# veronicaguerrini/BFQzip

Measured on AMD Instinct MI355X. Metric: Mbases/s end-to-end (eBWT+cluster+LF), reads and results resident in HBM, higher is better.
Workload: dtype u64

## Files before the change

bfqzip_amd/_lib.py:

```python
import ctypes as C
import os
import subprocess

_HERE = os.path.dirname(os.path.abspath(__file__))
LIB_PATH = os.path.join(_HERE, "libbfqhip.so")
_LIB = None

SYMBOLS = [
    "bfq_default_params", "bfq_create", "bfq_create_error", "bfq_destroy", "bfq_set_params",
    "bfq_last_error", "bfq_stream", "bfq_device_count", "bfq_pick_device", "bfq_device_lease", "bfq_device_release",
    "bfq_phase_enable", "bfq_phase", "bfq_phase_report", "bfq_output_prefault", "bfq_fastq_rows_estimate", "bfq_build_ebwt", "bfq_count_reads",
    "bfq_smooth_invert", "bfq_run_reads", "bfq_run_reads_device", "bfq_fetch_ebwt",
    "bfq_fastq_out_bound", "bfq_fastq_build_ebwt", "bfq_fastq_run", "bfq_fastq_run_streams",
    "bfq_smooth_invert_fastq", "bfq_fastq_run_job", "bfq_host_alloc", "bfq_host_free",
    "bfq_text_count_lines", "bfq_text_nth_newline", "bfq_file_put", "bfq_file_map", "bfq_file_unmap", "bfq_fastq_build_ebwt_fd", "bfq_smooth_invert_fastq_fd",
    "bfq_glob_begin", "bfq_glob_local_text", "bfq_glob_pile_counts", "bfq_glob_init_out", "bfq_glob_run_pile", "bfq_glob_finish",
    "bfq_synth_default", "bfq_synth_total", "bfq_synth_host", "bfq_synth_device", "bfq_synth_fastq",
    "bfq_posbin_geometry", "bfq_prof_enable", "bfq_prof_reset", "bfq_prof_count", "bfq_prof_get", "bfq_prof_trace_select", "bfq_prof_trace",
    "bfq_stream_bound", "bfq_stream_raw_len", "bfq_stream_compress", "bfq_stream_decompress",
    "bfq_stream_reserve", "bfq_stream_compress_device", "bfq_stream_ebwt_decode",
    "bfq_names_compress", "bfq_names_compress_device",
    "bfq_quals_compress", "bfq_quals_compress_device",
    "bfq_fastq_restore_bound", "bfq_fastq_restore", "bfq_fastq_restore_fd",
    "bfq_reorder_key", "bfq_fastq_reorder", "bfq_fastq_reorder_fd",
    "bfq_perm_bound", "bfq_perm_reads", "bfq_perm_encode", "bfq_perm_decode",
    "bfq_fastq_reorder_keep", "bfq_fastq_reorder_keep_fd", "bfq_fastq_unreorder", "bfq_fastq_unreorder_fd",
    "bfq_fastq_restore_ordered", "bfq_fastq_restore_ordered_fd",
    "bfq_fastq_restore_groups", "bfq_stream_members", "bfq_fastq_restore_grouped", "bfq_fastq_restore_grouped_fd",
    "bfq_fastq_compare", "bfq_fastq_compare_fd",
    "bfq_bgzf_probe", "bfq_bgzf_index", "bfq_bgzf_inflate", "bfq_bgzf_inflate_device", "bfq_bgzf_inflate_fd",
    "bfq_bgzf_deflate_bound", "bfq_bgzf_deflate_host", "bfq_bgzf_deflate", "bfq_bgzf_deflate_device", "bfq_bgzf_deflate_fd",
    "bfq_fastq_restore_bgzf_fd",
    "bfq_gzip_probe", "bfq_gzip_measure", "bfq_gzip_inflate", "bfq_gzip_inflate_device", "bfq_gzip_inflate_fd", "bfq_gzip_inflate_host",
    "bfq_gzip_host_error",
    "bfq_workspace_bytes", "bfq_version",
]


class Params(C.Structure):
    _fields_ = [(k, C.c_int32) for k in ("K", "m", "v", "f", "t", "term", "M", "B", "ext", "piles", "ws_cap_mib")] + \
               [("reserved", C.c_int32 * 5)]


class Stats(C.Structure):
    _fields_ = [(k, C.c_uint64) for k in (
        "num_clust", "num_clust_discarded", "num_clust_amb_discarded", "num_clust_mod",
        "num_clust_alleq", "bases_inside", "qs_smoothed", "modified",
        "n_rows", "n_reads", "n_segments", "n_big_segments")]

    def as_dict(self):
        return {k: int(getattr(self, k)) for k, _ in self._fields_}


class Synth(C.Structure):
    _fields_ = [("seed", C.c_uint64), ("N", C.c_uint64), ("Lmin", C.c_uint32), ("Lmax", C.c_uint32),
                ("coverage", C.c_uint32), ("err_ppm", C.c_uint32), ("n_ppm", C.c_uint32),
                ("snp_every", C.c_uint32), ("dsnp_every", C.c_uint32), ("both_strands", C.c_uint32),
                ("first", C.c_uint64), ("collection", C.c_uint64), ("reserved", C.c_uint32 * 2)]


MAX_PARTS = 4


class TextPart(C.Structure):
    _fields_ = [("data", C.c_void_p), ("len", C.c_uint64)]


class ReorderOpts(C.Structure):
    _fields_ = [("mode", C.c_int32), ("k", C.c_int32), ("seed", C.c_uint64), ("reserved", C.c_uint64 * 2)]


class RestoreGroup(C.Structure):
    _fields_ = [(k, C.c_uint64) for k in ("dna_off", "dna_len", "qs_off", "qs_len", "hdr_off", "hdr_len", "raw_stream", "raw_hdr",
                                          "reads", "text_bound")]


class BgzfMember(C.Structure):
    _fields_ = [("in_off", C.c_uint64), ("out_off", C.c_uint64), ("in_len", C.c_uint32), ("out_len", C.c_uint32)]


class GzipStats(C.Structure):
    _fields_ = [(k, C.c_uint64) for k in ("members", "pieces", "decoders", "chain", "skipped", "discarded")]

    def as_dict(self):
        return {k: int(getattr(self, k)) for k, _ in self._fields_}

    def __repr__(self):
        return "GzipStats(%s)" % ", ".join("%s=%d" % kv for kv in self.as_dict().items())


CMP_SYMS = 6
CMP_POS = 512


class CompareDiff(C.Structure):
    _fields_ = [("read", C.c_uint64), ("pos", C.c_uint32), ("base_a", C.c_uint8), ("base_b", C.c_uint8), ("qual_a", C.c_uint8), ("qual_b", C.c_uint8)]


COMPARE_SCALARS = ("n_reads", "total_bases", "n_diffs", "reads_changed", "reads_bases_changed", "reads_quals_changed", "bases_changed",
                   "quals_changed", "quals_raised", "quals_lowered", "qual_abs_sum", "qual_sq_sum", "qual_abs_max", "first_changed_read",
                   "headers_same", "headers_dropped", "headers_changed")
COMPARE_ARRAYS = (("subst", CMP_SYMS * CMP_SYMS), ("qual_hist_a", 256), ("qual_hist_b", 256), ("changed_base_qual_hist", 256),
                  ("pos_len", CMP_POS), ("pos_bases", CMP_POS), ("pos_quals", CMP_POS), ("pos_abs", CMP_POS))


class CompareReport(C.Structure):
    _fields_ = [(k, C.c_uint64) for k in COMPARE_SCALARS] + [(k, C.c_uint64 * n) for k, n in COMPARE_ARRAYS] + [("reserved", C.c_uint64 * 8)]


class FastqJob(C.Structure):
    _fields_ = [("parts", C.POINTER(TextPart)), ("nparts", C.c_int32), ("keep_headers", C.c_int32),
                ("out_fastq", C.c_void_p), ("cap_fastq", C.c_uint64),
                ("out_dna", C.c_void_p), ("out_qs", C.c_void_p), ("cap_stream", C.c_uint64),
                ("out_hdr", C.c_void_p), ("cap_hdr", C.c_uint64),
                ("fastq_len", C.c_uint64), ("stream_len", C.c_uint64), ("hdr_len", C.c_uint64),
                ("n_reads", C.c_uint64), ("total_bases", C.c_uint64),
                ("part_reads", C.c_uint64 * (MAX_PARTS + 1)), ("part_fastq_off", C.c_uint64 * (MAX_PARTS + 1)),
                ("part_stream_off", C.c_uint64 * (MAX_PARTS + 1)), ("part_hdr_off", C.c_uint64 * (MAX_PARTS + 1)),
                ("compress_streams", C.c_int32), ("name_codec", C.c_int32),
                ("dna_bytes", C.c_uint64), ("qs_bytes", C.c_uint64), ("hdr_bytes", C.c_uint64),
                ("qual_codec", C.c_int32), ("reserved1", C.c_int32)]


def build(clean=False):
    d = os.path.join(_HERE, "csrc")
    if clean:
        subprocess.check_call(["make", "-s", "-C", d, "clean"])
    subprocess.check_call(["make", "-s", "-j8", "-C", d, "all"])


def lib():
    global _LIB
    if _LIB is None:
        try:
            import torch
        except ImportError:
            pass
        if not os.path.exists(LIB_PATH):
            build()
        L = C.CDLL(LIB_PATH)
        L.bfq_create.restype = C.c_void_p
        L.bfq_create.argtypes = [C.c_int, C.POINTER(Params)]
        L.bfq_create_error.restype = C.c_char_p
        L.bfq_destroy.argtypes = [C.c_void_p]
        L.bfq_set_params.argtypes = [C.c_void_p, C.POINTER(Params)]
        L.bfq_last_error.restype = C.c_char_p
        L.bfq_last_error.argtypes = [C.c_void_p]
        L.bfq_stream.restype = C.c_void_p
        L.bfq_stream.argtypes = [C.c_void_p]
        L.bfq_version.restype = C.c_char_p
        L.bfq_workspace_bytes.restype = C.c_uint64
        L.bfq_workspace_bytes.argtypes = [C.c_void_p]
        L.bfq_synth_total.restype = C.c_uint64
        vp, u64 = C.c_void_p, C.c_uint64
        L.bfq_pick_device.argtypes = [C.c_char_p, C.c_int]
        L.bfq_device_lease.argtypes = [C.c_int, C.POINTER(C.c_char_p), C.c_int, C.c_char_p, C.c_int, C.POINTER(C.c_double)]
        L.bfq_device_release.argtypes = [C.c_int]
        L.bfq_phase_enable.argtypes = [C.c_int]
        L.bfq_phase.argtypes = [C.c_char_p]
        L.bfq_phase_report.argtypes = [C.c_char_p]
        L.bfq_output_prefault.argtypes = [C.c_int, u64, u64]
        L.bfq_fastq_rows_estimate.restype = u64
        L.bfq_fastq_rows_estimate.argtypes = [C.c_int, u64]
        L.bfq_build_ebwt.argtypes = [vp, vp, vp, vp, u64, C.c_int, vp, vp, vp]
        L.bfq_count_reads.argtypes = [vp, u64, C.c_int, C.POINTER(u64)]
        L.bfq_smooth_invert.argtypes = [vp, vp, vp, vp, C.c_int, u64, vp, vp, vp, C.POINTER(Stats)]
        L.bfq_run_reads.argtypes = [vp, vp, vp, vp, u64, vp, vp, C.POINTER(Stats)]
        L.bfq_run_reads_device.argtypes = [vp, vp, vp, vp, u64, u64, vp, vp, C.POINTER(Stats)]
        L.bfq_fetch_ebwt.argtypes = [vp, vp, vp, vp]
        L.bfq_fastq_out_bound.restype = C.c_uint64
        L.bfq_fastq_out_bound.argtypes = [u64, u64, u64]
        L.bfq_fastq_build_ebwt.argtypes = [vp, vp, u64, C.c_int, vp, vp, vp, u64, C.POINTER(u64), C.POINTER(u64)]
        L.bfq_fastq_run.argtypes = [vp, vp, u64, C.c_int, vp, u64, C.POINTER(u64), C.POINTER(Stats)]
        L.bfq_fastq_run_streams.argtypes = [vp, vp, u64, vp, vp, u64, C.POINTER(u64), vp, u64, C.POINTER(u64),
                                            C.POINTER(Stats)]
        L.bfq_smooth_invert_fastq.argtypes = [vp, vp, vp, vp, C.c_int, u64, vp, u64, vp, u64, C.POINTER(u64),
                                              C.POINTER(Stats)]
        L.bfq_fastq_run_job.argtypes = [vp, C.POINTER(FastqJob), C.POINTER(Stats)]
        L.bfq_glob_begin.argtypes = [vp, C.POINTER(TextPart), C.c_int, C.POINTER(u64), C.POINTER(u64)]
        L.bfq_glob_local_text.argtypes = [vp, vp, vp]
        L.bfq_glob_pile_counts.argtypes = [vp, vp, u64, vp]
        L.bfq_glob_init_out.argtypes = [vp, vp, vp, u64, vp, vp]
        L.bfq_glob_run_pile.argtypes = [vp, vp, vp, u64, C.c_int, C.c_int, vp, vp, C.POINTER(Stats)]
        L.bfq_glob_finish.argtypes = [vp, vp, vp, C.POINTER(FastqJob)]
        L.bfq_host_alloc.restype = vp
        L.bfq_host_alloc.argtypes = [u64]
        L.bfq_host_free.argtypes = [vp]
        L.bfq_text_count_lines.argtypes = [vp, u64, u64, vp, C.c_int]
        L.bfq_file_put.argtypes = [C.c_int, u64, vp, u64, C.c_int]
        L.bfq_file_map.restype = vp
        L.bfq_file_map.argtypes = [C.c_int, u64, u64, C.c_int]
        L.bfq_file_unmap.argtypes = [vp, u64, u64]
        L.bfq_text_nth_newline.restype = C.c_int64
        L.bfq_text_nth_newline.argtypes = [vp, u64, u64]
        L.bfq_synth_default.argtypes = [C.POINTER(Synth), u64, C.c_uint32]
        L.bfq_synth_total.argtypes = [C.POINTER(Synth)]
        L.bfq_synth_host.argtypes = [C.POINTER(Synth), vp, vp, vp]
        L.bfq_synth_device.argtypes = [vp, C.POINTER(Synth), vp, vp, vp]
        L.bfq_synth_fastq.argtypes = [vp, C.POINTER(Synth), vp, u64, C.POINTER(u64)]
        L.bfq_stream_bound.restype = u64
        L.bfq_stream_bound.argtypes = [u64]
        L.bfq_stream_raw_len.restype = C.c_int64
        L.bfq_stream_raw_len.argtypes = [vp, u64]
        L.bfq_stream_compress.argtypes = [vp, vp, u64, vp, u64, C.POINTER(u64)]
        L.bfq_stream_decompress.argtypes = [vp, vp, u64, vp, u64, C.POINTER(u64)]
        L.bfq_stream_reserve.argtypes = [vp, u64]
        L.bfq_names_compress.argtypes = [vp, vp, u64, C.c_uint32, vp, u64, C.POINTER(u64)]
        L.bfq_names_compress_device.argtypes = [vp, vp, u64, C.c_uint32, vp, u64, C.POINTER(u64)]
        L.bfq_quals_compress.argtypes = [vp, vp, u64, C.c_uint32, vp, u64, C.POINTER(u64)]
        L.bfq_quals_compress_device.argtypes = [vp, vp, u64, C.c_uint32, vp, u64, C.POINTER(u64)]
        L.bfq_stream_ebwt_decode.argtypes = [vp, vp, u64, vp, u64, vp, vp, u64, C.POINTER(u64), C.POINTER(u64)]
        L.bfq_fastq_restore_bound.restype = C.c_int64
        L.bfq_fastq_restore_bound.argtypes = [vp, u64, vp, u64, vp, u64]
        L.bfq_fastq_restore.argtypes = [vp, vp, u64, vp, u64, vp, u64, vp, u64, C.POINTER(u64), C.POINTER(u64)]
        L.bfq_fastq_restore_fd.argtypes = [vp, C.c_int, u64, C.c_int, u64, C.c_int, u64, C.c_int, C.POINTER(u64), C.POINTER(u64)]
        L.bfq_reorder_key.restype = u64
        L.bfq_reorder_key.argtypes = [vp, u64, C.c_int]
        L.bfq_fastq_reorder.argtypes = [vp, C.POINTER(TextPart), C.c_int, C.POINTER(ReorderOpts), C.POINTER(vp), C.POINTER(u64),
                                        C.POINTER(u64), vp, C.POINTER(u64)]
        L.bfq_fastq_reorder_fd.argtypes = [vp, C.POINTER(C.c_int), C.POINTER(u64), C.c_int, C.POINTER(ReorderOpts), C.POINTER(C.c_int),
                                           C.POINTER(u64), C.POINTER(u64)]
        pu64, pint = C.POINTER(u64), C.POINTER(C.c_int)
        L.bfq_perm_bound.restype = u64
        L.bfq_perm_bound.argtypes = [u64]
        L.bfq_perm_reads.restype = C.c_int64
        L.bfq_perm_reads.argtypes = [vp, u64]
        L.bfq_perm_encode.argtypes = [vp, u64, C.POINTER(ReorderOpts), vp, u64, pu64]
        L.bfq_perm_decode.argtypes = [vp, u64, vp, u64, pu64, C.POINTER(ReorderOpts), pu64]
        L.bfq_fastq_reorder_keep.argtypes = [vp, C.POINTER(TextPart), C.c_int, C.POINTER(ReorderOpts), C.POINTER(vp), pu64, pu64, vp, u64, pu64, pu64]
        L.bfq_fastq_reorder_keep_fd.argtypes = [vp, pint, pu64, C.c_int, C.POINTER(ReorderOpts), pint, C.c_int, pu64, pu64, pu64]
        L.bfq_fastq_unreorder.argtypes = [vp, C.POINTER(TextPart), C.c_int, vp, u64, C.POINTER(vp), pu64, pu64, pu64]
        L.bfq_fastq_unreorder_fd.argtypes = [vp, pint, pu64, C.c_int, C.c_int, u64, pint, pu64, pu64]
        L.bfq_fastq_restore_ordered.argtypes = [vp, vp, u64, vp, u64, vp, u64, vp, u64, vp, u64, pu64, pu64]
        L.bfq_fastq_restore_ordered_fd.argtypes = [vp, C.c_int, u64, C.c_int, u64, C.c_int, u64, C.c_int, u64, C.c_int, pu64, pu64]
        L.bfq_fastq_restore_groups.restype = C.c_int64
        L.bfq_fastq_restore_groups.argtypes = [vp, u64, vp, u64, vp, u64, C.POINTER(RestoreGroup), u64, C.c_char_p, C.c_int]
        L.bfq_stream_members.restype = C.c_int64
        L.bfq_stream_members.argtypes = [vp, u64]
        L.bfq_fastq_restore_grouped.argtypes = [vp, vp, u64, vp, u64, vp, u64, u64, u64, vp, u64, pu64, pu64]
        L.bfq_fastq_restore_grouped_fd.argtypes = [vp, C.c_int, u64, C.c_int, u64, C.c_int, u64, u64, u64, C.c_int, pu64, pu64]
        L.bfq_stream_compress_device.argtypes = [vp, vp, u64, vp, u64, C.POINTER(u64)]
        L.bfq_fastq_compare.argtypes = [vp, C.POINTER(TextPart), C.c_int, C.POINTER(TextPart), C.c_int, vp, u64, C.POINTER(CompareReport), vp, u64]
        L.bfq_fastq_compare_fd.argtypes = [vp, C.c_int, u64, C.c_int, u64, C.c_int, u64, C.POINTER(CompareReport), vp, u64]
        L.bfq_bgzf_probe.argtypes = [vp, u64]
        L.bfq_bgzf_index.argtypes = [vp, u64, C.POINTER(BgzfMember), u64, pu64, pu64, pu64]
        L.bfq_bgzf_inflate.argtypes = [vp, vp, u64, vp, u64, pu64]
        L.bfq_bgzf_inflate_device.argtypes = [vp, vp, u64, vp, u64, pu64]
        L.bfq_bgzf_inflate_fd.argtypes = [vp, C.c_int, u64, C.c_int, pu64]
        L.bfq_bgzf_deflate_bound.restype = u64
        L.bfq_bgzf_deflate_bound.argtypes = [u64]
        L.bfq_bgzf_deflate_host.argtypes = [vp, u64, C.c_int, vp, u64, pu64]
        L.bfq_bgzf_deflate.argtypes = [vp, vp, u64, C.c_int, vp, u64, pu64]
        L.bfq_bgzf_deflate_device.argtypes = [vp, vp, u64, C.c_int, vp, u64, pu64]
        L.bfq_bgzf_deflate_fd.argtypes = [vp, C.c_int, u64, C.c_int, C.c_int, pu64]
        pgs = C.POINTER(GzipStats)
        L.bfq_gzip_probe.argtypes = [vp, u64]
        L.bfq_gzip_measure.argtypes = [vp, vp, u64, u64, pu64, pu64, pgs]
        L.bfq_gzip_inflate.argtypes = [vp, vp, u64, u64, vp, u64, pu64, pgs]
        L.bfq_gzip_inflate_device.argtypes = [vp, vp, u64, u64, vp, u64, pu64, pgs]
        L.bfq_gzip_inflate_fd.argtypes = [vp, C.c_int, u64, u64, C.c_int, pu64, pgs]
        L.bfq_gzip_inflate_host.argtypes = [vp, u64, u64, vp, u64, pu64, pgs]
        L.bfq_gzip_host_error.restype = C.c_char_p
        L.bfq_gzip_host_error.argtypes = []
        L.bfq_fastq_restore_bgzf_fd.argtypes = [vp, C.c_int, u64, C.c_int, u64, C.c_int, u64, C.c_int, u64, C.c_int, C.c_int, pu64, pu64, pu64]
        L.bfq_posbin_geometry.argtypes = [u64, C.POINTER(u64), C.POINTER(C.c_int)]
        L.bfq_prof_enable.argtypes = [vp, C.c_int]
        L.bfq_prof_reset.argtypes = [vp]
        L.bfq_prof_count.argtypes = [vp]
        L.bfq_prof_trace_select.argtypes = [vp, C.c_int]
        L.bfq_prof_trace.restype = C.c_int64
        L.bfq_prof_trace.argtypes = [vp, vp, u64]
        L.bfq_prof_get.argtypes = [vp, C.c_int, C.c_char_p, C.c_int, C.POINTER(C.c_double),
                                   C.POINTER(u64), C.POINTER(C.c_double)]
        _LIB = L
    return _LIB
```

bfqzip_amd/csrc/bfq_api.hip:

```cpp
#include <math.h>
#include <time.h>
#include <stdlib.h>
#include <stdio.h>
#include <string.h>
#include <unistd.h>
#include <errno.h>
#include <algorithm>
#include <new>
#include "bfq_internal.h"
#include "bfq_synth.h"
#include "bfq_device.h"
#include "bfq_rank.h"
#include "bfq_posbin.h"

const char *const BFQ_KERNEL_NAMES[K_NUM] = {
    "k_text_from_reads", "k_pack3", "k_build_keys", "k_radix_hist", "k_scan", "k_radix_scatter", "k_huge_round",
    "k_cluster_big", "k_refine_chunk", "k_refine_big", "k_emit_bwt", "k_lf_count", "k_lf_build", "k_lcp_flags",
    "k_cluster", "k_invert_count", "k_invert", "k_synth", "k_fastq", "k_bfs", "k_codec", "misc",
    "k_restore_index", "k_fq_format_lines", "k_reorder_keys", "k_reorder_gather",
    "k_fq_format_ordered", "k_perm_pack", "k_perm_invert", "k_posbin_l1", "k_posbin_l2", "k_posbin_apply",
    "k_cmp_check", "k_cmp_compare", "k_cmp_emit", "k_bgzf_inflate", "k_bgzf_deflate"};

static thread_local std::string g_createErr;

void bfq_ctx::reserveBegin(size_t bytes)
{
    bytes = (bytes + 0xFFFFF) & ~(size_t)0xFFFFF;
    if (wsThread || bytes <= ws.cap || (wsLimit() && bytes > wsLimit())) return;
    wsPendBytes = bytes; wsPend = nullptr;
    const int dev = device;
    wsThread = new std::thread([this, dev, bytes] {
        struct timespec t0, t1;
        clock_gettime(CLOCK_MONOTONIC, &t0);
        void *p = nullptr;
        if (hipSetDevice(dev) != hipSuccess || hipMalloc(&p, bytes) != hipSuccess) { (void)hipGetLastError(); p = nullptr; }
        clock_gettime(CLOCK_MONOTONIC, &t1);
        wsPend = (char *)p;
        wsPendSecs = (t1.tv_sec - t0.tv_sec) + 1e-9 * (t1.tv_nsec - t0.tv_nsec);
    });
}
void bfq_ctx::reserveJoin(bool adopt, size_t need)
{
    if (!wsThread) return;
    wsThread->join();
    delete wsThread;
    wsThread = nullptr;
    if (!wsPend) return;
    if (adopt && need <= wsPendBytes && need > ws.cap && !(wsLimit() && wsPendBytes > wsLimit())) {
        adoptWorkspace(wsPend, wsPendBytes);
        if (bfq_env().trace) fprintf(stderr, "[bfq] workspace %.1f GiB: hipMalloc %.3f s, beside the upload\n", ws.cap / 1073741824.0, wsPendSecs);
    } else (void)hipFree(wsPend);
    wsPend = nullptr; wsPendBytes = 0;
}
void bfq_ctx::wsFree() { adoptWorkspace(nullptr, 0); }
void bfq_ctx::adoptWorkspace(char *p, size_t bytes)
{
    if (ws.base) { quiesce(); (void)hipFree(ws.base); }
    ws = Arena{p, bytes, 0, ws.peak};
}

void bfq_ctx::reserve(size_t bytes)
{
    bytes = (bytes + 0xFFFFF) & ~(size_t)0xFFFFF;
    reserveJoin(true, bytes);
    if (wsLimit() && bytes > wsLimit()) {
        char b[200];
        snprintf(b, sizeof b, "device workspace of %.1f GiB is above the cap of %.1f GiB (bfq_params.ws_cap_mib / BFQ_WS_CAP)", bytes / 1073741824.0, wsLimit() / 1073741824.0);
        throw BfqError{BFQ_E_NOMEM, b};
    }
    if (bytes > ws.cap || (wsLimit() && ws.cap > wsLimit())) {
        wsFree();
        struct timespec t0, t1;
        clock_gettime(CLOCK_MONOTONIC, &t0);
        char *p = nullptr;
        const hipError_t e = hipMalloc((void **)&p, bytes);
        clock_gettime(CLOCK_MONOTONIC, &t1);
        if (bfq_env().trace) fprintf(stderr, "[bfq] workspace %.1f GiB: hipMalloc %.3f s\n", bytes / 1073741824.0, (t1.tv_sec - t0.tv_sec) + 1e-9 * (t1.tv_nsec - t0.tv_nsec));
        if (e != hipSuccess) {
            char b[160];
            snprintf(b, sizeof b, "device workspace of %zu bytes: %s", bytes, hipGetErrorString(e));
            (void)hipGetLastError();
            throw BfqError{BFQ_E_NOMEM, b};
        }
        adoptWorkspace(p, bytes);
    }
    ws.release(0);
    d_bwt = d_qual = nullptr; d_lcp = nullptr; d_gcnt = nullptr; n = N = 0;
}
void bfq_ctx::dropWorkspace()
{
    wsFree();
    d_bwt = d_qual = nullptr; d_lcp = nullptr; d_gcnt = nullptr;
}
void bfq_ctx::profBegin(int id, double bytes)
{
    if (!profOn) return;
    if (evUsed + 2 > evPool.size()) {
        size_t old = evPool.size();
        evPool.resize(old + 256);
        for (size_t i = old; i < evPool.size(); i++) HIP_CHECK(hipEventCreate(&evPool[i]));
    }
    ProfRec r{id, evPool[evUsed], evPool[evUsed + 1], bytes};
    evUsed += 2;
    HIP_CHECK(hipEventRecord(r.a, stream));
    recs.push_back(r);
}
void bfq_ctx::profEnd()
{
    if (!profOn) return;
    HIP_CHECK(hipEventRecord(recs.back().b, stream));
}
void bfq_ctx::profCollect()
{
    for (auto &r : recs) {
        float ms = 0;
        if (hipEventElapsedTime(&ms, r.a, r.b) == hipSuccess) {
            profMs[r.id] += ms; profLaunches[r.id]++; profBytes[r.id] += r.bytes;
            if (r.id == profTraceId && profTrace.size() < (1u << 20)) profTrace.push_back(ms);
        }
    }
    recs.clear();
    evUsed = 0;
}
void bfq_ctx::sync() { HIP_CHECK(hipStreamSynchronize(stream)); }
void bfq_ctx::zeroCounters() { HIP_CHECK(hipMemsetAsync(d_cnt, 0, sizeof(DevCounters), stream)); }
void bfq_ctx::fetchCounters()
{
    HIP_CHECK(hipMemcpyAsync(&h_cnt, d_cnt, sizeof(DevCounters), hipMemcpyDeviceToHost, stream));
    sync();
}

static int host_q(double x) { return (int)round(-10 * log10(x)); }

extern "C" void bfq_default_params(bfq_params *p)
{
    memset(p, 0, sizeof(*p));
    p->K = 16; p->m = 2; p->v = '>'; p->f = 40; p->t = 20; p->term = '#'; p->M = 2; p->B = 0; p->ext = 0; p->piles = 0;
}
extern "C" const char *bfq_create_error(void) { return g_createErr.c_str(); }
extern "C" const char *bfq_version(void) { return "bfqzip_amd 0.1 (gfx950)"; }
extern "C" int bfq_device_count(void)
{
    int nd = 0;
    if (hipGetDeviceCount(&nd) != hipSuccess) { (void)hipGetLastError(); return 0; }
    return nd;
}

extern "C" int bfq_pick_device(char *info, int info_cap)
{
    const BfqEnv &E = bfq_env();
    int real = 0;
    if (hipGetDeviceCount(&real) != hipSuccess || real < 1) { (void)hipGetLastError(); return BFQ_E_HIP; }
    const int slots = E.fakeDevices > 0 ? E.fakeDevices : real;
    if (E.device >= slots) return BFQ_E_ARG;
    if (!E.lease) {
        const int d = E.device >= 0 ? E.device % real : 0;
        if (info && info_cap > 0) snprintf(info, info_cap, "device %d (no lease)", d);
        return d;
    }
    std::vector<std::string> ids(slots);
    std::vector<const char *> idp(slots);
    for (int k = 0; k < slots; k++) {
        char bus[64] = {0};
        if (E.fakeDevices > 0) ids[k] = "fake" + std::to_string(k) + "of" + std::to_string(slots);
        else if (hipDeviceGetPCIBusId(bus, sizeof bus, k) == hipSuccess && bus[0]) ids[k] = std::string("gpu-") + bus;
        else { (void)hipGetLastError(); ids[k] = "gpu-index" + std::to_string(k); }
        idp[k] = ids[k].c_str();
    }
    char path[256] = {0};
    double waited = 0;
    const int slot = bfq_device_lease(slots, idp.data(), E.device, path, sizeof path, &waited);
    if (slot < 0) return slot;
    if (info && info_cap > 0) snprintf(info, info_cap, "device %d lease %s waited %.3f s", slot % real, path, waited);
    return slot % real;
}

extern "C" bfq_ctx *bfq_create(int device, const bfq_params *p)
{
    bfq_ctx *c = nullptr;
    try {
        int nd = 0;
        if (hipGetDeviceCount(&nd) != hipSuccess || nd == 0)
            throw BfqError{BFQ_E_HIP, "no HIP device available (libbfqhip.so has no CPU fallback)"};
        if (device < 0 || device >= nd) throw BfqError{BFQ_E_ARG, "device index out of range"};
        c = new bfq_ctx();
        c->device = device;
        if (p) c->P = *p; else bfq_default_params(&c->P);
        c->env = bfq_env_read();
        HIP_CHECK(hipSetDevice(device));
        HIP_CHECK(hipStreamCreateWithFlags(&c->stream, hipStreamNonBlocking));
        HIP_CHECK(hipMalloc((void **)&c->d_cnt, sizeof(DevCounters)));
        memset(c->profMs, 0, sizeof c->profMs); memset(c->profLaunches, 0, sizeof c->profLaunches);
        memset(c->profBytes, 0, sizeof c->profBytes);
        g_bfqHipStarted = true;
        double pw[256];
        for (int q = 0; q < 256; q++) pw[q] = pow(10, -((double)(signed char)q - 33) / 10);
        c->qthrLo = -170; c->qthrN = 311;
        std::vector<double> thr(c->qthrN);
        for (int k = 0; k < c->qthrN; k++) {
            int q = c->qthrLo + k;
            double xlo = 1e-30, xhi = 1e30;
            u64 lo, hi;
            memcpy(&lo, &xlo, 8); memcpy(&hi, &xhi, 8);
            while (hi - lo > 1) {
                u64 mid = lo + (hi - lo) / 2;
                double xm; memcpy(&xm, &mid, 8);
                if (host_q(xm) <= q) hi = mid; else lo = mid;
            }
            memcpy(&thr[k], &hi, 8);
        }
        HIP_CHECK(hipMalloc((void **)&c->d_powtab, sizeof pw));
        HIP_CHECK(hipMalloc((void **)&c->d_qthr, sizeof(double) * c->qthrN));
        HIP_CHECK(hipMemcpy(c->d_powtab, pw, sizeof pw, hipMemcpyHostToDevice));
        HIP_CHECK(hipMemcpy(c->d_qthr, thr.data(), sizeof(double) * c->qthrN, hipMemcpyHostToDevice));
        return c;
    } catch (const BfqError &e) {
        g_createErr = e.msg;
    } catch (const std::exception &e) {
        g_createErr = e.what();
    }
    delete c;
    return nullptr;
}

extern "C" void bfq_destroy(bfq_ctx *c)
{
    if (!c) return;
    (void)hipSetDevice(c->device);
    if (c->stream) (void)hipStreamSynchronize(c->stream);
    for (auto e : c->evPool) (void)hipEventDestroy(e);
    c->ioFree();
    if (c->d_text) (void)hipFree(c->d_text);
    if (bfq_env().trace && c->ws.cap) fprintf(stderr, "[bfq] workspace: %.1f GiB reserved, %.1f GiB used at the peak\n", c->ws.cap / 1073741824.0, c->ws.peak / 1073741824.0);
    c->wsFree();
    if (c->d_cnt) (void)hipFree(c->d_cnt);
    if (c->d_powtab) (void)hipFree(c->d_powtab);
    if (c->d_qthr) (void)hipFree(c->d_qthr);
    if (c->copyStream) (void)hipStreamDestroy(c->copyStream);
    if (c->stream) (void)hipStreamDestroy(c->stream);
    delete c;
}
extern "C" int bfq_set_params(bfq_ctx *c, const bfq_params *p)
{
    if (!c || !p) return BFQ_E_ARG;
    c->P = *p;
    c->env = bfq_env_read();
    return BFQ_OK;
}
extern "C" const char *bfq_last_error(bfq_ctx *c) { return c ? c->err.c_str() : "null context"; }
extern "C" void *bfq_stream(bfq_ctx *c) { return c ? (void *)c->stream : nullptr; }
extern "C" uint64_t bfq_workspace_bytes(bfq_ctx *c) { return c ? c->ws.cap : 0; }
extern "C" int bfq_prof_enable(bfq_ctx *c, int on) { if (!c) return BFQ_E_ARG; c->profOn = on != 0; return BFQ_OK; }
extern "C" void bfq_prof_reset(bfq_ctx *c)
{
    if (!c) return;
    memset(c->profMs, 0, sizeof c->profMs); memset(c->profLaunches, 0, sizeof c->profLaunches);
    memset(c->profBytes, 0, sizeof c->profBytes);
    c->profTrace.clear();
}
extern "C" int bfq_prof_trace_select(bfq_ctx *c, int idx)
{
    if (!c || idx < -1 || idx >= K_NUM) return BFQ_E_ARG;
    c->profTraceId = idx; c->profTrace.clear();
    return BFQ_OK;
}
extern "C" int64_t bfq_prof_trace(bfq_ctx *c, float *ms, uint64_t cap)
{
    if (!c) return BFQ_E_ARG;
    const size_t k = std::min<size_t>(cap, c->profTrace.size());
    if (ms && k) memcpy(ms, c->profTrace.data(), k * sizeof(float));
    return (int64_t)c->profTrace.size();
}
extern "C" int bfq_prof_count(bfq_ctx *c) { (void)c; return K_NUM; }
extern "C" int bfq_posbin_geometry(uint64_t n_rows, uint64_t *window, int *bin_shift)
{
    const int s = bfq_posbin_shift(n_rows);
    if (window) *window = BFQ_PB_W;
    if (bin_shift) *bin_shift = s;
    return s >= 0 ? BFQ_OK : BFQ_E_ARG;
}
extern "C" int bfq_prof_get(bfq_ctx *c, int idx, char *name, int cap, double *ms, uint64_t *launches, double *bytes)
{
    if (!c || idx < 0 || idx >= K_NUM) return BFQ_E_ARG;
    if (name && cap > 0) { strncpy(name, BFQ_KERNEL_NAMES[idx], cap - 1); name[cap - 1] = 0; }
    if (ms) *ms = c->profMs[idx];
    if (launches) *launches = c->profLaunches[idx];
    if (bytes) *bytes = c->profBytes[idx];
    return BFQ_OK;
}

static void check_counters(bfq_ctx *c)
{
    const DevCounters &h = c->h_cnt;
    if (h.errSymbol) throw BfqError{BFQ_E_SYMBOL, "symbol outside {A,C,G,T,N,terminator}"};
    if (h.errTooLong) throw BfqError{BFQ_E_TOO_LONG, "read longer than BFQ_MAX_READ_LEN"};
    if (h.errInvert) throw BfqError{BFQ_E_NOT_EBWT, "LF walk did not close: not an eBWT of a read collection"};
    if (h.mismatch) throw BfqError{BFQ_E_NOT_EBWT, "eBWT is not in #_i<#_j<A<C<G<N<T suffix order"};
    if (h.errFreq3) throw BfqError{BFQ_E_FREQ3, "three frequent symbols in a cluster (bfq_int.cpp:505 assert); raise -f"};
}
static void finish_call(bfq_ctx *c, bfq_stats *st = nullptr)
{
    c->fetchCounters();
    c->profCollect();
    check_counters(c);
    if (!st) return;
    const u64 *s = c->h_cnt.stats;
    st->num_clust = s[0]; st->num_clust_discarded = s[1]; st->num_clust_amb_discarded = s[2];
    st->num_clust_mod = s[3]; st->num_clust_alleq = s[4]; st->bases_inside = s[5];
    st->qs_smoothed = s[6]; st->modified = s[7];
    st->n_rows = c->n; st->n_reads = c->N;
    st->n_segments = c->h_cnt.nSegs; st->n_big_segments = c->h_cnt.bigTotal + c->h_cnt.bigCount;
}

static size_t ws_need(u64 n, u64 N, u64 extra)
{
    const u64 nb = ceil_div(n + 1, bfq_radix_block_elems(n)) + 8;
    size_t need = 0;
    need += 4 * (n + 256) + 24 * (n / 256 + 2) + 4096;
    need += 8 * bfq_t3_alloc(n / 21 + 3);
    need += 6 * 4 * (n + 256);
    need += 256 * nb * 12 + (nb + 4096) * 64;
    need += 16 * (N + 64);
    need += extra + (64u << 20);
    return need;
}

static size_t ws_need_given(u64 n, u64 N, u64 extra)
{
    size_t need = 0;
    need += 6 * (n + 256) + 4096;
    const size_t table = 10 * (n + 1024) + 72 * (n / 256 + 2);
    need += table > extra ? table : extra;
    need += 16 * (N + 64) + (n >> 20) * 64 + 4096;
    need += 64u << 20;
    return need;
}

static size_t ws_need_capped(u64 n, u64 N, u64 pile, u64 extra)
{
    size_t need = 0;
    need += 4 * (n + 512) + 8 * bfq_t3_alloc(n / 21 + 3);
    need += 2 * 6 * 12 * (n / 32768 + 2) + 16 * (N + 64);
    if (pile) need += 32 * (pile + 256) + 256 * 12 * (ceil_div(pile + 1, bfq_radix_block_elems(pile)) + 8200) + (pile / 32768 + 4096) * 64;
    need += extra + (96u << 20);
    return need;
}

static void reserve_step1(bfq_ctx *c, u64 n, u64 N, u64 extra, bool allowCapped = true)
{
    int mode = c->P.piles;
    if (c->env.piles) mode = c->env.piles;
    if (mode == 2 && !allowCapped) mode = 1;
    const u64 cap = n / 10 * 3 + (1u << 20);
    if (mode <= 0) {
        try { c->reserve(ws_need(n, N, extra)); return; }
        catch (const BfqError &e) { if (mode < 0 || e.code != BFQ_E_NOMEM) throw; }
    }
    if (mode != 2) {
        try { c->reserve(bfq_ws_need_piles(n, N, cap, extra)); c->call.piles = true; return; }
        catch (const BfqError &e) { if (e.code != BFQ_E_NOMEM || !c->wsLimit() || !allowCapped) throw; }
    }
    const size_t base = ws_need_capped(n, N, 0, extra), lim = c->wsLimit();
    u64 rows = !lim ? n / 4 + (1u << 20) : lim > base + (128u << 20) ? (u64)((lim - base - (128u << 20)) / 32) : 0;
    if (rows > n / 4 + (1u << 20)) rows = n / 4 + (1u << 20);
    if (lim && rows < n / 64 + 4096) {
        char b[220];
        snprintf(b, sizeof b, "workspace cap of %.1f GiB too small for %llu rows: the capped mode needs %.1f GiB + 32 bytes per row of its largest two-symbol pile",
                 lim / 1073741824.0, (unsigned long long)n, base / 1073741824.0);
        throw BfqError{BFQ_E_NOMEM, b};
    }
    c->reserve(ws_need_capped(n, N, rows, extra));
    c->call.capped = true; c->call.cappedPileRows = rows;
}

void bfq_step1_device(bfq_ctx *c, const u8 *d_bases, const u8 *d_quals, const u64 *d_roff, u64 N, u64 total,
                      int termOut, bfq_stats *st)
{
    if (c->call.piles) { bfq_step1_piles(c, d_bases, d_quals, d_roff, N, total, termOut, st); return; }
    u64 n = total + N;
    if (n >= (1ull << BFQ_POS_BITS)) throw BfqError{BFQ_E_ARG, "collection too large (2^37 rows)"};
    c->n = n; c->N = N;
    c->d_bwt = c->call.extBwt ? c->call.extBwt : c->alloc<u8>(n + 64);
    c->d_qual = c->call.extQual ? c->call.extQual : c->alloc<u8>(n + 64);
    c->d_lcp = c->alloc<u16>(n + 64);
    c->d_gcnt = c->alloc<u32>(6 * (n / 256 + 1));
    c->gcntTerm = termOut & 0xFF;
    if (!n) return;
    size_t m0 = c->mark();
    u64 nwords = n / BFQ_SYMS_PER_WORD + 3;
    u64 *text3 = c->alloc<u64>(bfq_t3_alloc(nwords));
    SortRec A, B;
    A.w12 = c->alloc<u64>(n + 16);
    const size_t mKeep = c->mark();
    A.w0 = c->alloc<u32>(n + 16);
    const size_t mB = c->mark();
    B.w0 = c->alloc<u32>(n + 16);
    B.w12 = c->alloc<u64>(n + 16);
    if (bfq_env().trace) fprintf(stderr, "[bfq] sort buffers: A.w12 %p A.w0 %p B.w0 %p B.w12 %p (arena %p)\n", (void *)A.w12, (void *)A.w0, (void *)B.w0, (void *)B.w12, (void *)c->ws.base);
    u8 *T8 = (u8 *)A.w0, *Q8 = (u8 *)A.w12;
    bfq_build_text(c, d_bases, d_quals, d_roff, N, n, T8, Q8, text3, nwords);
    u32 *hist0 = c->alloc<u32>(256 * ceil_div(n, bfq_radix_block_elems(n)));
    static_assert(BFQ_KEY_PASSES & 1, "an odd number of passes ends in the other buffer");
    bfq_build_keys(c, T8, Q8, text3, n, B, hist0);
    bfq_radix_sort(c, B, A, n, BFQ_KEY_PASSES, hist0);
    c->release(mB);
    bfq_refine(c, A, text3, n, c->d_lcp, st);
    bfq_emit_bwt(c, A, n, termOut, c->d_bwt, c->d_qual, c->d_gcnt);
    if (c->call.keepRecs) { c->release(mKeep); c->call.d_w12 = A.w12; c->call.d_text3 = text3; c->call.keepMark = m0; }
    else c->release(m0);
    if (c->call.onRows) c->call.onRows(0, n);
}

static void count_lengths(bfq_ctx *c, const RankIndex &R, u64 *d_roff, u32 *lens)
{
    const u64 n = c->n, N = c->N;
    bfq_invert_count(c, R, N, lens);
    bfq_exscan_u32(c, lens, d_roff, N, d_roff + N);
    u64 tot2 = 0;
    HIP_CHECK(hipMemcpyAsync(&tot2, d_roff + N, 8, hipMemcpyDeviceToHost, c->stream));
    c->fetchCounters();
    check_counters(c);
    if (tot2 != n - N) throw BfqError{BFQ_E_NOT_EBWT, "LF walks do not cover the eBWT"};
}
struct StreamOut { u8 *h_dna, *h_qs; bool packed = false; };
static void invert_lines(bfq_ctx *c, const RankIndex &R, const u64 *d_roff, u8 *d_dna, u8 *d_qs, const StreamOut *so)
{
    const u64 N = c->N;
    const bool lines = !so->packed;
    const bool pinned = (!so->h_dna || bfq_is_pinned(so->h_dna)) && (!so->h_qs || bfq_is_pinned(so->h_qs));
    const int C = (pinned && N >= (1u << 16) && !c->env.noOverlap) ? 8 : 1;
    if (C == 1) {
        bfq_invert(c, R, N, d_roff, c->P.B, d_dna, d_qs, 0, ~0ull, lines);
        const u64 sl = (c->n - N) + (lines ? N : 0);
        if (so->h_dna) bfq_download(c, so->h_dna, d_dna, sl);
        if (so->h_qs) bfq_download(c, so->h_qs, d_qs, sl);
        return;
    }
    const hipStream_t cs = c->copy();
    u64 first[9], off[9];
    for (int j = 0; j <= C; j++) first[j] = N * (u64)j / C;
    for (int j = 0; j <= C; j++) HIP_CHECK(hipMemcpyAsync(&off[j], d_roff + first[j], 8, hipMemcpyDeviceToHost, c->stream));
    c->sync();
    ScopedEvent ev[8];
    for (int j = 0; j < C; j++) {
        bfq_invert(c, R, N, d_roff, c->P.B, d_dna, d_qs, first[j], first[j + 1] - first[j], lines);
        HIP_CHECK(hipEventRecord(ev[j], c->stream));
        HIP_CHECK(hipStreamWaitEvent(cs, ev[j], 0));
        const u64 b0 = off[j] + (lines ? first[j] : 0), b1 = off[j + 1] + (lines ? first[j + 1] : 0);
        if (so->h_dna) HIP_CHECK(hipMemcpyAsync(so->h_dna + b0, d_dna + b0, b1 - b0, hipMemcpyDeviceToHost, cs));
        if (so->h_qs) HIP_CHECK(hipMemcpyAsync(so->h_qs + b0, d_qs + b0, b1 - b0, hipMemcpyDeviceToHost, cs));
    }
    HIP_CHECK(hipStreamSynchronize(cs));
}
struct EbwtOut { u8 *sym, *qual, *patch; u8 *lineDna, *lineQs; };
__global__ __launch_bounds__(256) void k_ebwt_rows(const u64 *__restrict__ lfq, u64 n, u32 term, int B, u8 *__restrict__ sym, u8 *__restrict__ qual,
                                                   u8 *__restrict__ patch)
{
    for (u64 r = (u64)blockIdx.x * blockDim.x + threadIdx.x; r < n; r += (u64)gridDim.x * blockDim.x) {
        const u64 x = lfq[r];
        const u32 code = lfq_replaced(x) ? lfq_repl(x) : lfq_code(x);
        sym[r] = code ? bfq_code_sym(code) : (u8)term;
        patch[r] = lfq_replaced(x) ? bfq_code_sym(lfq_code(x)) : (u8)0;
        const u32 q = lfq_qual(x);
        qual[r] = lfq_code(x) ? (u8)(B ? bfq_bin8(q) : q) : (u8)'!';
    }
}
static void steps234_device(bfq_ctx *c, u64 *d_roff, u8 *d_out_bases, u8 *d_out_quals, u32 *lens = nullptr, const StreamOut *so = nullptr,
                            const EbwtOut *eo = nullptr)
{
    u64 n = c->n, N = c->N;
    if (!n) return;
    const u32 *gc = (c->d_gcnt && c->gcntTerm == (c->P.term & 0xFF)) ? c->d_gcnt : nullptr;
    RankIndex R = bfq_rank_build(c, c->d_bwt, c->d_qual, n, c->P.term, gc);
    bool guessed = false;
    if (lens) {
        if (N && (n - N) % N == 0 && !c->env.noLengthGuess) { bfq_fixed_offsets(c, N, (n - N) / N, d_roff); guessed = true; }
        else count_lengths(c, R, d_roff, lens);
    }
    u8 *in = c->alloc<u8>(n + 64);
    bfq_lcp_flags(c, c->d_lcp, n, c->P.K, in);
    bfq_clusters(c, R, c->d_bwt, c->d_qual, in, n);
    if (eo) {
        KLAUNCH(c, K_MISC, 10.0 * (double)n, k_ebwt_rows, bfq_grid(n, 256), 256, (const u64 *)R.lfq, n, (u32)(c->P.term & 0xFF), c->P.B, eo->sym, eo->qual, eo->patch);
        if (eo->lineQs) { StreamOut none{nullptr, nullptr}; invert_lines(c, R, d_roff, eo->lineDna, eo->lineQs, &none); }
        return;
    }
    auto walk = [&] { if (so) invert_lines(c, R, d_roff, d_out_bases, d_out_quals, so); else bfq_invert(c, R, N, d_roff, c->P.B, d_out_bases, d_out_quals); };
    walk();
    if (guessed) {
        c->fetchCounters();
        if (c->h_cnt.errInvert) {
            HIP_CHECK(hipMemsetAsync(&c->d_cnt->errInvert, 0, sizeof(u64), c->stream));
            count_lengths(c, R, d_roff, lens);
            walk();
        }
    }
}

__global__ __launch_bounds__(256) void k_lines_init(const u8 *__restrict__ bases, const u8 *__restrict__ quals, const u64 *__restrict__ roff, u64 N,
                                                    int B, u8 *__restrict__ dna, u8 *__restrict__ qs)
{
    const u32 sub = threadIdx.x & 15u;
    const u64 ngrp = ((u64)gridDim.x * blockDim.x) >> 4;
    for (u64 i = ((u64)blockIdx.x * blockDim.x + threadIdx.x) >> 4; i < N; i += ngrp) {
        const u64 b = roff[i], len = roff[i + 1] - b, o = b + i;
        for (u64 k = sub; k < len; k += 16) { dna[o + k] = bases[b + k]; const u32 q = quals[b + k]; qs[o + k] = (u8)(B ? bfq_bin8(q) : q); }
        if (sub == 0) { dna[o + len] = 10; qs[o + len] = 10; }
    }
}
__global__ __launch_bounds__(256) void k_lines_strip(const u8 *__restrict__ dna, const u8 *__restrict__ qs, const u64 *__restrict__ roff, u64 N,
                                                     u8 *__restrict__ bases, u8 *__restrict__ quals)
{
    const u32 sub = threadIdx.x & 15u;
    const u64 ngrp = ((u64)gridDim.x * blockDim.x) >> 4;
    for (u64 i = ((u64)blockIdx.x * blockDim.x + threadIdx.x) >> 4; i < N; i += ngrp) {
        const u64 b = roff[i], len = roff[i + 1] - b, o = b + i;
        for (u64 k = sub; k < len; k += 16) { bases[b + k] = dna[o + k]; quals[b + k] = qs[o + k]; }
    }
}
static void steps34_positions(bfq_ctx *c, const u8 *d_bases, const u8 *d_quals, const u64 *d_roff, u8 *d_out_bases, u8 *d_out_quals)
{
    const u64 n = c->n, N = c->N;
    if (!n) return;
    u8 *dna = c->alloc<u8>(n + 64), *qs = c->alloc<u8>(n + 64);
    if (N) KLAUNCH(c, K_MISC, 4.0 * (double)(n - N), k_lines_init, bfq_grid(N, 16), 256, d_bases, d_quals, d_roff, N, c->P.B, dna, qs);
    u8 *in = c->alloc<u8>(n + 64);
    bfq_lcp_flags(c, c->d_lcp, n, c->P.K, in);
    ClusterPos pm{c->call.d_w12, c->call.d_text3, dna, qs, c->P.B};
    RankIndex none{nullptr, n};
    bfq_clusters(c, none, c->d_bwt, c->d_qual, in, n, &pm);
    if (N) KLAUNCH(c, K_MISC, 4.0 * (double)(n - N), k_lines_strip, bfq_grid(N, 16), 256, (const u8 *)dna, (const u8 *)qs, d_roff, N, d_out_bases, d_out_quals);
}

static size_t posbins_room_needed(u64 n)
{
    const size_t pb = bfq_posbins_need(n);
    if (pb == ~(size_t)0) return pb;
    return pb + 3 * (n + 64 + 256) + 24 * (n / 256 + 8) + (1u << 20);
}
static void steps34_posbins(bfq_ctx *c, const u64 *d_roff, u8 *d_out_bases, u8 *d_out_quals)
{
    const u64 n = c->n, N = c->N;
    if (!n) return;
    u8 *editQual = c->alloc<u8>(n + 64), *repl = c->alloc<u8>(n + 64);
    HIP_CHECK(hipMemcpyAsync(editQual, c->d_qual, n, hipMemcpyDeviceToDevice, c->stream));
    HIP_CHECK(hipMemsetAsync(repl, 0, n + 64, c->stream));
    {
        const size_t mk = c->mark();
        u8 *in = c->alloc<u8>(n + 64);
        bfq_lcp_flags(c, c->d_lcp, n, c->P.K, in);
        ClusterPos pm{c->call.d_w12, c->call.d_text3, nullptr, nullptr, c->P.B, editQual, repl};
        RankIndex none{nullptr, n};
        bfq_clusters(c, none, c->d_bwt, c->d_qual, in, n, &pm);
        c->release(mk);
    }
    bfq_posbins(c, const_cast<u64 *>(c->call.d_w12), repl, editQual, n, d_roff, N, c->P.B, d_out_bases, d_out_quals);
}

static void steps_capped(bfq_ctx *c, const u8 *d_bases, const u8 *d_quals, const u64 *d_roff, u64 N, u64 total, u8 *dna, u8 *qs)
{
    const u64 n = total + N;
    if (n >= (1ull << BFQ_POS_BITS)) throw BfqError{BFQ_E_ARG, "collection too large (2^37 rows)"};
    c->n = n; c->N = N;
    c->d_bwt = c->d_qual = nullptr; c->d_lcp = nullptr; c->d_gcnt = nullptr;
    if (!n) return;
    if (c->P.K < 1) throw BfqError{BFQ_E_NOMEM, "the capped mode needs -k >= 1 (with -k 0 every row is in one cluster): raise the workspace cap"};
    const size_t m0 = c->mark();
    const u64 nwords = n / BFQ_SYMS_PER_WORD + 3;
    u64 *text3 = c->alloc<u64>(bfq_t3_alloc(nwords));
    u8 *T8 = c->alloc<u8>(n + 64), *Q8 = c->alloc<u8>(n + 64);
    bfq_build_text(c, d_bases, d_quals, d_roff, N, n, T8, Q8, text3, nwords);
    if (N) KLAUNCH(c, K_MISC, 4.0 * (double)(n - N), k_lines_init, bfq_grid(N, 16), 256, d_bases, d_quals, d_roff, N, c->P.B, dna, qs);
    u64 cnt[36];
    bfq_pile_pair_counts(c, T8, n, cnt);
    c->fetchCounters();
    if (c->h_cnt.errSymbol || c->h_cnt.errTooLong) { c->release(m0); return; }
    const bool two = c->P.K >= 2;
    for (u32 s = 1; s <= 5; s++) {
        for (u32 s2 = two ? 1u : 7u; s2 <= (two ? 5u : 7u); s2++) {
            u64 rows = 0;
            if (two) rows = cnt[6 * s + s2]; else for (int q = 0; q < 6; q++) rows += cnt[6 * s + q];
            if (!rows) continue;
            if (rows > c->call.cappedPileRows) {
                char b[220];
                snprintf(b, sizeof b, "pile '%c%c' holds %llu rows, the workspace cap leaves room for %llu: raise bfq_params.ws_cap_mib / BFQ_WS_CAP",
                         "#ACGNT"[s], two ? "#ACGNT"[s2] : '*', (unsigned long long)rows, (unsigned long long)c->call.cappedPileRows);
                throw BfqError{BFQ_E_NOMEM, b};
            }
            const size_t mp = c->mark();
            PileRows pr;
            if (bfq_env().trace) fprintf(stderr, "[bfq capped] pile %c%c: %llu rows, arena %zu of %zu used\n", "#ACGNT"[s], two ? "#ACGNT"[s2] : '*', (unsigned long long)rows, c->ws.top, c->ws.cap);
            const u64 m = bfq_run_one_pile(c, T8, Q8, text3, n, s, s2, c->P.term & 0xFF, &pr);
            if (bfq_env().trace) { c->sync(); fprintf(stderr, "[bfq capped]   sorted + refined\n"); }
            if (m) {
                u8 *in = c->alloc<u8>(m + 64);
                bfq_lcp_flags(c, pr.lcp, m, c->P.K, in);
                ClusterPos pm{pr.w12, text3, dna, qs, c->P.B};
                RankIndex none{nullptr, m};
                bfq_clusters(c, none, pr.bwt, pr.qs, in, m, &pm);
            }
            c->sync();
            if (bfq_env().trace) fprintf(stderr, "[bfq capped]   clusters done\n");
            c->release(mp);
        }
    }
    c->release(m0);
}
static void run_capped_reads(bfq_ctx *c, const u8 *bases, const u8 *quals, const u64 *roff, u64 N, u64 total, u8 *ob, u8 *oq)
{
    u8 *dna = c->alloc<u8>(total + N + 64), *qs = c->alloc<u8>(total + N + 64);
    steps_capped(c, bases, quals, roff, N, total, dna, qs);
    if (N) KLAUNCH(c, K_MISC, 4.0 * (double)total, k_lines_strip, bfq_grid(N, 16), 256, (const u8 *)dna, (const u8 *)qs, roff, N, ob, oq);
}

extern "C" int bfq_run_reads_device(bfq_ctx *c, const uint8_t *d_bases, const uint8_t *d_quals,
                                    const uint64_t *d_read_off, uint64_t N, uint64_t total, uint8_t *d_out_bases,
                                    uint8_t *d_out_quals, bfq_stats *st)
{
    return guarded(c, [&] {
        if (st) memset(st, 0, sizeof *st);
        reserve_step1(c, total + N, N, 0);
        c->zeroCounters();
        const u64 *roff = (const u64 *)d_read_off;
        const bool fused = !c->call.capped && !c->call.piles;
        const bool posBins = fused && !c->env.posMode && c->env.posBins && bfq_posbin_shift(total + N) >= 0;
        c->call.keepRecs = fused && (c->env.posMode || posBins);
        if (c->call.capped) run_capped_reads(c, d_bases, d_quals, roff, N, total, d_out_bases, d_out_quals);
        else {
            bfq_step1_device(c, d_bases, d_quals, roff, N, total, c->P.term, st);
            if (posBins && total + N && c->ws.room() < posbins_room_needed(total + N)) {
                c->release(c->call.keepMark);
                c->call.keepRecs = false;
            }
            if (c->call.keepRecs && posBins) steps34_posbins(c, roff, d_out_bases, d_out_quals);
            else if (c->call.keepRecs) steps34_positions(c, d_bases, d_quals, roff, d_out_bases, d_out_quals);
            else steps234_device(c, (u64 *)d_read_off, d_out_bases, d_out_quals);
        }
        finish_call(c, st);
    });
}

extern "C" int bfq_run_reads(bfq_ctx *c, const uint8_t *h_bases, const uint8_t *h_quals, const uint64_t *h_read_off,
                             uint64_t N, uint8_t *h_out_bases, uint8_t *h_out_quals, bfq_stats *st)
{
    return guarded(c, [&] {
        if (st) memset(st, 0, sizeof *st);
        if (!h_read_off) throw BfqError{BFQ_E_ARG, "null read offsets"};
        u64 total = h_read_off[N];
        reserve_step1(c, total + N, N, 6 * (total + 256) + 10 * (N + 64));
        c->zeroCounters();
        u8 *db = c->alloc<u8>(total + 64), *dq = c->alloc<u8>(total + 64);
        u8 *ob = c->alloc<u8>(total + 64), *oq = c->alloc<u8>(total + 64);
        u64 *dr = c->alloc<u64>(N + 1);
        bfq_upload(c, db, h_bases, total);
        bfq_upload(c, dq, h_quals, total);
        bfq_upload(c, dr, h_read_off, 8 * (N + 1));
        if (c->call.capped) run_capped_reads(c, db, dq, dr, N, total, ob, oq);
        else {
            bfq_step1_device(c, db, dq, dr, N, total, c->P.term, st);
            steps234_device(c, dr, ob, oq);
        }
        bfq_download(c, h_out_bases, ob, total);
        bfq_download(c, h_out_quals, oq, total);
        finish_call(c, st);
    });
}

extern "C" int bfq_build_ebwt(bfq_ctx *c, const uint8_t *h_bases, const uint8_t *h_quals, const uint64_t *h_read_off,
                              uint64_t N, int term_out, uint8_t *h_bwt, uint8_t *h_bwtqs, uint16_t *h_lcp16)
{
    return guarded(c, [&] {
        if (!h_read_off) throw BfqError{BFQ_E_ARG, "null read offsets"};
        u64 total = h_read_off[N], n = total + N;
        reserve_step1(c, n, N, 2 * (total + 256) + 8 * (N + 64), false);
        c->zeroCounters();
        u8 *db = c->alloc<u8>(total + 64), *dq = c->alloc<u8>(total + 64);
        u64 *dr = c->alloc<u64>(N + 1);
        bfq_upload(c, db, h_bases, total);
        bfq_upload(c, dq, h_quals, total);
        bfq_upload(c, dr, h_read_off, 8 * (N + 1));
        bfq_step1_device(c, db, dq, dr, N, total, term_out, nullptr);
        if (h_bwt) bfq_download(c, h_bwt, c->d_bwt, n);
        if (h_bwtqs) bfq_download(c, h_bwtqs, c->d_qual, n);
        if (h_lcp16) bfq_download(c, h_lcp16, c->d_lcp, 2 * n);
        finish_call(c);
    });
}

extern "C" int bfq_fetch_ebwt(bfq_ctx *c, uint8_t *h_bwt, uint8_t *h_qs, uint16_t *h_lcp16)
{
    return guarded(c, [&] {
        if (!c->d_bwt) throw BfqError{BFQ_E_ARG, "no eBWT resident"};
        if (h_bwt) HIP_CHECK(hipMemcpyAsync(h_bwt, c->d_bwt, c->n, hipMemcpyDeviceToHost, c->stream));
        if (h_qs) HIP_CHECK(hipMemcpyAsync(h_qs, c->d_qual, c->n, hipMemcpyDeviceToHost, c->stream));
        if (h_lcp16) HIP_CHECK(hipMemcpyAsync(h_lcp16, c->d_lcp, 2 * c->n, hipMemcpyDeviceToHost, c->stream));
        c->sync();
    });
}

__global__ __launch_bounds__(256) void k_lcp_widen(const u8 *__restrict__ raw, int lb, u64 n, u16 *__restrict__ out)
{
    for (u64 i = (u64)blockIdx.x * blockDim.x + threadIdx.x; i < n; i += (u64)gridDim.x * blockDim.x) {
        u64 v = lb == 1 ? raw[i] : lb == 2 ? ((const u16 *)raw)[i] : ((const u32 *)raw)[i];
        out[i] = (u16)(v > 0xFFFE ? 0xFFFE : v);
    }
}

// ... 873 lines not shown
```

bfqzip_amd/csrc/bfq_device.h:

```cpp
#pragma once
#include <hip/hip_runtime.h>
#include "bfq_common.h"

#define BFQ_WAVE 64

__device__ __forceinline__ u32 bfq_lane() { return __builtin_amdgcn_mbcnt_hi(~0u, __builtin_amdgcn_mbcnt_lo(~0u, 0u)); }
__device__ __forceinline__ u64 bfq_lanemask_lt() { return (1ull << bfq_lane()) - 1ull; }

__device__ __forceinline__ u64 bfq_readlane64(u64 v, int srcLane)
{
    u32 lo = (u32)__builtin_amdgcn_readlane((int)(u32)v, srcLane);
    u32 hi = (u32)__builtin_amdgcn_readlane((int)(u32)(v >> 32), srcLane);
    return ((u64)hi << 32) | lo;
}
__device__ __forceinline__ u64 bfq_permute64(u64 v, int dstLane)
{
    u32 lo = (u32)__builtin_amdgcn_ds_permute(dstLane << 2, (int)(u32)v);
    u32 hi = (u32)__builtin_amdgcn_ds_permute(dstLane << 2, (int)(u32)(v >> 32));
    return ((u64)hi << 32) | lo;
}

__device__ __forceinline__ void bfq_wave_sync()
{
    __builtin_amdgcn_fence(__ATOMIC_RELEASE, "wavefront");
    __builtin_amdgcn_wave_barrier();
    __builtin_amdgcn_fence(__ATOMIC_ACQUIRE, "wavefront");
}

__device__ __forceinline__ u64 bfq_from_next_lane(u64 v)
{
    u32 lo = (u32)__builtin_amdgcn_update_dpp(0, (int)(u32)v, 0x130, 0xF, 0xF, true);
    u32 hi = (u32)__builtin_amdgcn_update_dpp(0, (int)(u32)(v >> 32), 0x130, 0xF, 0xF, true);
    return ((u64)hi << 32) | lo;
}
__device__ __forceinline__ u64 bfq_from_prev_lane(u64 v)
{
    u32 lo = (u32)__builtin_amdgcn_update_dpp(0, (int)(u32)v, 0x138, 0xF, 0xF, true);
    u32 hi = (u32)__builtin_amdgcn_update_dpp(0, (int)(u32)(v >> 32), 0x138, 0xF, 0xF, true);
    return ((u64)hi << 32) | lo;
}

#define BFQ_DPP_ROW_SHR(v, k) __builtin_amdgcn_update_dpp(0, (int)(v), 0x110 + (k), 0xF, 0xF, true)
__device__ __forceinline__ u32 bfq_wave_incscan32(u32 v)
{
    v += (u32)BFQ_DPP_ROW_SHR(v, 1);
    v += (u32)BFQ_DPP_ROW_SHR(v, 2);
    v += (u32)BFQ_DPP_ROW_SHR(v, 4);
    v += (u32)BFQ_DPP_ROW_SHR(v, 8);
    const u32 t0 = (u32)__builtin_amdgcn_readlane((int)v, 15), t1 = (u32)__builtin_amdgcn_readlane((int)v, 31),
              t2 = (u32)__builtin_amdgcn_readlane((int)v, 47);
    const u32 row = bfq_lane() >> 4;
    return v + (row >= 1 ? t0 : 0u) + (row >= 2 ? t1 : 0u) + (row >= 3 ? t2 : 0u);
}
__device__ __forceinline__ u64 bfq_row_shr64(u64 v, int k)
{
    u32 lo, hi;
    switch (k) {
    case 1: lo = (u32)BFQ_DPP_ROW_SHR((u32)v, 1); hi = (u32)BFQ_DPP_ROW_SHR((u32)(v >> 32), 1); break;
    case 2: lo = (u32)BFQ_DPP_ROW_SHR((u32)v, 2); hi = (u32)BFQ_DPP_ROW_SHR((u32)(v >> 32), 2); break;
    case 4: lo = (u32)BFQ_DPP_ROW_SHR((u32)v, 4); hi = (u32)BFQ_DPP_ROW_SHR((u32)(v >> 32), 4); break;
    default: lo = (u32)BFQ_DPP_ROW_SHR((u32)v, 8); hi = (u32)BFQ_DPP_ROW_SHR((u32)(v >> 32), 8); break;
    }
    return ((u64)hi << 32) | lo;
}
__device__ __forceinline__ u64 bfq_wave_incscan64(u64 v)
{
    v += bfq_row_shr64(v, 1);
    v += bfq_row_shr64(v, 2);
    v += bfq_row_shr64(v, 4);
    v += bfq_row_shr64(v, 8);
    const u64 t0 = bfq_readlane64(v, 15), t1 = bfq_readlane64(v, 31), t2 = bfq_readlane64(v, 47);
    const u32 row = bfq_lane() >> 4;
    return v + (row >= 1 ? t0 : 0ull) + (row >= 2 ? t1 : 0ull) + (row >= 3 ? t2 : 0ull);
}

__device__ __forceinline__ u32 bfq_wave_incscan32_bp(u32 v)
{
    u32 lane = bfq_lane();
#pragma unroll
    for (int d = 1; d < 64; d <<= 1) {
        u32 t = (u32)__builtin_amdgcn_ds_bpermute(((int)lane - d) << 2, (int)v);
        if ((int)lane >= d) v += t;
    }
    return v;
}

__device__ __forceinline__ u64 bfq_block_exscan64(u64 v, u64 *sh, u64 *total)
{
    u32 lane = bfq_lane(), w = threadIdx.x >> 6;
    u64 inc = bfq_wave_incscan64(v);
    if (lane == 63) sh[w] = inc;
    __syncthreads();
    u64 s0 = sh[0], s1 = sh[1], s2 = sh[2], s3 = sh[3];
    u64 base = (w > 0 ? s0 : 0) + (w > 1 ? s1 : 0) + (w > 2 ? s2 : 0);
    *total = s0 + s1 + s2 + s3;
    __syncthreads();
    return base + inc - v;
}
__device__ __forceinline__ u32 bfq_block_exscan32(u32 v, u32 *sh, u32 *total)
{
    u32 lane = bfq_lane(), w = threadIdx.x >> 6;
    u32 inc = bfq_wave_incscan32(v);
    if (lane == 63) sh[w] = inc;
    __syncthreads();
    u32 s0 = sh[0], s1 = sh[1], s2 = sh[2], s3 = sh[3];
    u32 base = (w > 0 ? s0 : 0) + (w > 1 ? s1 : 0) + (w > 2 ? s2 : 0);
    *total = s0 + s1 + s2 + s3;
    __syncthreads();
    return base + inc - v;
}
```

bfqzip_amd/csrc/bfq_host.cpp:

```cpp
#include <errno.h>
#include <fcntl.h>
#include <stdio.h>
#include <stdlib.h>
#include <string.h>
#include <sched.h>
#include <sys/file.h>
#include <sys/mman.h>
#include <sys/stat.h>
#include <time.h>
#include <unistd.h>
#include <algorithm>
#include <atomic>
#include <condition_variable>
#include <mutex>
#include <string>
#include <thread>
#include <vector>
#include "bfq_internal_host.h"
#include "bfq_reorder.h"
#include "bfq_perm.h"
#include "bfq_bgzf.h"

static double now_s()
{
    struct timespec ts;
    clock_gettime(CLOCK_MONOTONIC, &ts);
    return ts.tv_sec + 1e-9 * ts.tv_nsec;
}

BfqEnv bfq_env_read()
{
    {
        BfqEnv e;
        auto geti = [](const char *k, int dflt) { const char *v = getenv(k); return (v && *v) ? atoi(v) : dflt; };
        auto getu = [](const char *k, unsigned long long dflt) {
            const char *v = getenv(k);
            if (!v || !*v) return dflt;
            char *end = nullptr;
            double x = strtod(v, &end);
            if (end && (*end == 'G' || *end == 'g')) x *= 1073741824.0;
            else if (end && (*end == 'M' || *end == 'm')) x *= 1048576.0;
            else if (end && (*end == 'K' || *end == 'k')) x *= 1024.0;
            return (unsigned long long)x;
        };
        e.trace = getenv("BFQ_TRACE") != nullptr;
        e.piles = getenv("BFQ_PILES") ? (atoi(getenv("BFQ_PILES")) == 2 ? 2 : atoi(getenv("BFQ_PILES")) ? 1 : -1) : 0;
        e.pilesSplit = getenv("BFQ_PILES_SPLIT") != nullptr;
        e.noOverlap = getenv("BFQ_NO_OVERLAP") != nullptr;
        e.noLengthGuess = getenv("BFQ_NO_LENGTH_GUESS") != nullptr;
        e.posMode = geti("BFQ_POSMODE", 0) != 0;
        e.posBins = geti("BFQ_POSBINS", 1) != 0;
        e.ioThreads = geti("BFQ_IO_THREADS", 0);
        e.prefaultThreads = geti("BFQ_PREFAULT_THREADS", -1);
        e.hugeCap = getu("BFQ_HUGE_CAP", 0);
        e.wsCap = getu("BFQ_WS_CAP", 0);
        e.device = getenv("BFQ_DEVICE") ? atoi(getenv("BFQ_DEVICE")) : -1;
        e.fakeDevices = geti("BFQ_FAKE_DEVICES", 0);
        e.lease = geti("BFQ_LEASE", 1) != 0;
        if (const char *d = getenv("BFQ_LEASE_DIR")) e.leaseDir = d;
        e.noOutmap = getenv("BFQ_NO_OUTMAP") != nullptr;
        e.compact = geti("BFQ_COMPACT", 0) != 0;
        e.prefaultPause = geti("BFQ_PREFAULT_PAUSE", 0) != 0;
        e.compactWin = getu("BFQ_COMPACT_WIN", 0);
        e.compactRing = getu("BFQ_COMPACT_RING", 0);
        e.bgzfBatch = getu("BFQ_BGZF_BATCH", 0);
        e.dnaStatic = geti("BFQ_DNA_STATIC", 0);
        e.dnacK = geti("BFQ_DNAC_K", 0); e.dnacH = geti("BFQ_DNAC_H", 0); e.dnacW = geti("BFQ_DNAC_W", 0); e.dnacSkip = geti("BFQ_DNAC_TSKIP", -1);
        return e;
    }
}
const BfqEnv &bfq_env()
{
    static const BfqEnv E = bfq_env_read();
    return E;
}

int bfq_cpu_budget()
{
    static const int budget = [] {
        int n = (int)std::thread::hardware_concurrency();
        cpu_set_t set;
        if (sched_getaffinity(0, sizeof set, &set) == 0) { const int k = CPU_COUNT(&set); if (k > 0 && (n <= 0 || k < n)) n = k; }
        for (const char *path : {"/sys/fs/cgroup/cpu.max", "/sys/fs/cgroup/cpu/cpu.cfs_quota_us"}) {
            FILE *f = fopen(path, "r");
            if (!f) continue;
            char a[64] = {0}, b[64] = {0};
            const int got = fscanf(f, "%63s %63s", a, b);
            fclose(f);
            if (got >= 1 && strcmp(a, "max") != 0) {
                double quota = atof(a), period = got >= 2 ? atof(b) : 100000.0;
                if (got < 2) {
                    FILE *g = fopen("/sys/fs/cgroup/cpu/cpu.cfs_period_us", "r");
                    if (g) { if (fscanf(g, "%lf", &period) != 1) period = 100000.0; fclose(g); }
                }
                if (quota > 0 && period > 0) { const int k = (int)(quota / period + 0.5); if (k >= 1 && (n <= 0 || k < n)) n = k; }
            }
            break;
        }
        return n > 0 ? n : 1;
    }();
    return budget;
}

namespace {
struct Held { int slot; int fd; std::string path; };
std::mutex g_leaseMu;
std::vector<Held> g_held;

std::string lease_dir()
{
    const BfqEnv &E = bfq_env();
    if (!E.leaseDir.empty()) return E.leaseDir;
    if (access("/dev/shm", W_OK | X_OK) == 0) return "/dev/shm";
    return "/tmp";
}
}

extern "C" int bfq_device_lease(int n_slots, const char *const *slot_ids, int only_slot, char *path_out, int path_cap,
                                double *waited_s)
{
    if (n_slots < 1) return BFQ_E_ARG;
    if (only_slot >= n_slots) return BFQ_E_ARG;
    const std::string dir = lease_dir();
    std::vector<int> fds(n_slots, -1);
    std::vector<std::string> paths(n_slots);
    const mode_t um = umask(0);
    for (int k = 0; k < n_slots; k++) {
        if (only_slot >= 0 && k != only_slot) continue;
        std::string id = (slot_ids && slot_ids[k]) ? slot_ids[k] : ("slot" + std::to_string(k));
        for (auto &ch : id) if (!((ch >= '0' && ch <= '9') || (ch >= 'a' && ch <= 'z') || (ch >= 'A' && ch <= 'Z') || ch == '.' || ch == '-')) ch = '_';
        paths[k] = dir + "/bfqzip_amd." + id + ".lock";
        fds[k] = open(paths[k].c_str(), O_RDWR | O_CREAT | O_CLOEXEC, 0666);
    }
    umask(um);
    int got = -1;
    const double t0 = now_s();
    unsigned spin = 0;
    bool any = false;
    for (int k = 0; k < n_slots; k++) any = any || fds[k] >= 0;
    if (!any) return BFQ_E_IO;
    while (got < 0) {
        for (int k = 0; k < n_slots && got < 0; k++) {
            if (fds[k] < 0) continue;
            if (flock(fds[k], LOCK_EX | LOCK_NB) == 0) got = k;
            else if (errno != EWOULDBLOCK && errno != EINTR) { close(fds[k]); fds[k] = -1; }
        }
        if (got >= 0) break;
        any = false;
        for (int k = 0; k < n_slots; k++) any = any || fds[k] >= 0;
        if (!any) return BFQ_E_IO;
        const unsigned us = spin < 20 ? 2000 : spin < 100 ? 10000 : 50000;
        usleep(us);
        spin++;
    }
    for (int k = 0; k < n_slots; k++)
        if (k != got && fds[k] >= 0) close(fds[k]);
    if (waited_s) *waited_s = now_s() - t0;
    if (path_out && path_cap > 0) { strncpy(path_out, paths[got].c_str(), path_cap - 1); path_out[path_cap - 1] = 0; }
    {
        char b[64];
        int l = snprintf(b, sizeof b, "%ld\n", (long)getpid());
        if (ftruncate(fds[got], 0) == 0) { ssize_t w = pwrite(fds[got], b, (size_t)l, 0); (void)w; }
    }
    std::lock_guard<std::mutex> g(g_leaseMu);
    g_held.push_back(Held{got, fds[got], paths[got]});
    return got;
}

extern "C" int bfq_device_release(int slot)
{
    std::lock_guard<std::mutex> g(g_leaseMu);
    for (size_t i = 0; i < g_held.size(); i++)
        if (g_held[i].slot == slot) {
            flock(g_held[i].fd, LOCK_UN);
            close(g_held[i].fd);
            g_held.erase(g_held.begin() + (long)i);
            return BFQ_OK;
        }
    return BFQ_E_ARG;
}

namespace {
struct Phase { std::string name; double secs; };
std::mutex g_phMu;
std::vector<Phase> g_phases;
double g_phT0 = 0, g_phLast = 0;
int g_phCur = -1;
bool g_phOn = false;
double g_startAge = -1;

double process_age()
{
    FILE *f = fopen("/proc/self/stat", "r");
    if (!f) return -1;
    char buf[2048];
    size_t r = fread(buf, 1, sizeof buf - 1, f);
    fclose(f);
    buf[r] = 0;
    const char *p = strrchr(buf, ')');
    if (!p) return -1;
    p++;
    unsigned long long start = 0;
    int field = 3;
    while (*p && field < 22) { while (*p == ' ') p++; while (*p && *p != ' ') p++; field++; }
    if (sscanf(p, " %llu", &start) != 1) return -1;
    double up = 0;
    f = fopen("/proc/uptime", "r");
    if (!f) return -1;
    int ok = fscanf(f, "%lf", &up);
    fclose(f);
    if (ok != 1) return -1;
    const long hz = sysconf(_SC_CLK_TCK);
    return up - (double)start / (double)(hz > 0 ? hz : 100);
}
}

extern "C" void bfq_phase_enable(int on)
{
    std::lock_guard<std::mutex> g(g_phMu);
    g_phOn = on != 0;
}
extern "C" void bfq_phase(const char *name)
{
    std::lock_guard<std::mutex> g(g_phMu);
    const double t = now_s();
    if (g_phCur < 0 && g_phases.empty()) { g_phT0 = t; g_phLast = t; g_startAge = process_age(); }
    if (g_phCur >= 0) g_phases[(size_t)g_phCur].secs += t - g_phLast;
    g_phLast = t;
    g_phCur = -1;
    if (!name) return;
    for (size_t i = 0; i < g_phases.size(); i++)
        if (g_phases[i].name == name) g_phCur = (int)i;
    if (g_phCur < 0) { g_phases.push_back(Phase{name, 0}); g_phCur = (int)g_phases.size() - 1; }
}
extern "C" void bfq_phase_report(const char *tool)
{
    bfq_phase(nullptr);
    std::lock_guard<std::mutex> g(g_phMu);
    if (g_phases.empty() || !(g_phOn || bfq_env().trace)) return;
    std::string s = "[bfq phases] {\"tool\": \"";
    s += tool ? tool : "";
    s += "\"";
    char b[128];
    if (g_startAge >= 0) { snprintf(b, sizeof b, ", \"exec_to_main\": %.3f", g_startAge); s += b; }
    for (auto &p : g_phases) { snprintf(b, sizeof b, ", \"%s\": %.3f", p.name.c_str(), p.secs); s += b; }
    snprintf(b, sizeof b, ", \"total\": %.3f}", (g_startAge >= 0 ? g_startAge : 0) + (g_phLast - g_phT0));
    s += b;
    fprintf(stderr, "%s\n", s.c_str());
    fflush(stderr);
}

struct bfq_outmap {
    int fd = -1;
    char *map = nullptr;
    uint64_t mapLen = 0;
    std::vector<std::thread> th;
    std::atomic<uint64_t> next{0};
    std::atomic<bool> stop{false};
    std::atomic<int> alive{0};
    std::atomic<uint64_t> preEnd{0};
    std::atomic<uint64_t> done{0};
    uint64_t nslices = 0;
    std::atomic<bool> noFallocate{false};
    bool holdForHip = false;
    std::atomic<uint64_t> fallocDone{0};
    std::atomic<bool> fallocRunning{false};
    std::thread fallocThread;
    std::atomic<bool> failed{false};
    double tOpen = 0, tHelpersDone = 0;
    std::atomic<uint8_t> *state = nullptr;
};
static const uint64_t PF_SLICE = 32ull << 20;

namespace {
std::mutex g_popMu;
std::condition_variable g_popCv;
int g_popBusy = 0;
struct PopSlot {
    PopSlot()
    {
        int lim = bfq_env().prefaultThreads;
        if (lim <= 0) lim = 2;
        std::unique_lock<std::mutex> lk(g_popMu);
        g_popCv.wait(lk, [&] { return g_popBusy < lim; });
        g_popBusy++;
    }
    ~PopSlot() { std::lock_guard<std::mutex> g(g_popMu); g_popBusy--; g_popCv.notify_one(); }
};
}
std::atomic<int> g_bfqUploadsRunning{0};
static void populate_slice(bfq_outmap *m, uint64_t idx)
{
    const uint64_t b = idx * PF_SLICE, e = std::min<uint64_t>(b + PF_SLICE, m->mapLen);
    if (m->failed.load()) return;
    while (!m->noFallocate.load() && !m->failed.load() && m->fallocDone.load() < e) {
        if (m->fallocRunning.load() && e <= m->preEnd.load()) { usleep(200); continue; }
        if (fallocate(m->fd, 0, (off_t)b, (off_t)(e - b)) != 0) {
            if (errno == ENOSPC || errno == EDQUOT || errno == EFBIG) { m->failed = true; return; }
            m->noFallocate = true;
        }
        break;
    }
    if (m->failed.load()) return;
    PopSlot slot;
#ifdef MADV_POPULATE_WRITE
    if (madvise(m->map + b, (size_t)(e - b), MADV_POPULATE_WRITE) != 0) {
        if (errno == ENOMEM || errno == EFAULT || errno == ENOSPC) { m->failed = true; return; }
        if (errno != EINVAL) { m->failed = true; return; }
    }
#endif
    m->done += e - b;
}
static void hold_for_hip(bfq_outmap *m);
static void falloc_worker(bfq_outmap *m)
{
    hold_for_hip(m);
    const uint64_t STEP = 128ull << 20;
    for (uint64_t b = 0;;) {
        if (m->stop.load(std::memory_order_relaxed) || m->failed.load()) break;
        if (bfq_env().prefaultPause && g_bfqUploadsRunning.load(std::memory_order_relaxed) > 0) { usleep(500); continue; }
        const uint64_t pe = m->preEnd.load();
        if (b >= pe) break;
        const uint64_t e = std::min<uint64_t>(b + STEP, std::min<uint64_t>(pe + PF_SLICE, m->mapLen));
        if (fallocate(m->fd, 0, (off_t)b, (off_t)(e - b)) != 0) {
            if (errno == ENOSPC || errno == EDQUOT || errno == EFBIG) m->failed = true; else m->noFallocate = true;
            break;
        }
        m->fallocDone = e;
        b = e;
    }
    m->fallocRunning = false;
}
std::atomic<bool> g_bfqHipStarted{false};
static void hold_for_hip(bfq_outmap *m)
{
    if (m->holdForHip)
        for (double t0 = now_s(); !g_bfqHipStarted.load(std::memory_order_relaxed) && !m->stop.load(std::memory_order_relaxed) && now_s() - t0 < 3.0;) usleep(1000);
}
static void prefault_worker(bfq_outmap *m)
{
    hold_for_hip(m);
    for (;;) {
        if (m->stop.load(std::memory_order_relaxed)) break;
        const uint64_t idx = m->next.fetch_add(1);
        if (idx >= m->nslices || idx * PF_SLICE >= m->preEnd.load()) { m->next.fetch_sub(1); break; }
        uint8_t z = 0;
        if (m->state[idx].compare_exchange_strong(z, 1)) { populate_slice(m, idx); m->state[idx].store(2); }
    }
    if (--m->alive == 0) m->tHelpersDone = now_s();
}
bool bfq_outmap_ensure(bfq_outmap *m, uint64_t off, uint64_t len)
{
    if (!m || !len) return true;
    if (m->failed.load()) return false;
// ... 248 lines not shown
```

bfqzip_amd/csrc/bfq_internal.h:

```cpp
#pragma once
#include <stdlib.h>
#include <errno.h>
#include <unistd.h>
#include <hip/hip_runtime.h>
#include <stdint.h>
#include <functional>
#include <new>
#include <optional>
#include <string>
#include <vector>
#include <thread>
#include "../../include/bfqzip_hip.h"
#include "bfq_common.h"
#include "bfq_internal_host.h"
#include "bfq_arena.h"

#define HIP_CHECK(expr)                                                                        \
    do {                                                                                       \
        hipError_t e__ = (expr);                                                               \
        if (e__ != hipSuccess)                                                                 \
            throw BfqError{BFQ_E_HIP, std::string(#expr) + ": " + hipGetErrorString(e__)};     \
    } while (0)

enum BfqKernel {
    K_TEXT = 0, K_PACK, K_KEYS, K_RADIX_HIST, K_SCAN, K_RADIX_SCATTER, K_HUGE_ROUND, K_CLUSTER_BIG,
    K_REFINE_WAVE, K_REFINE_BIG, K_EMIT, K_RANK_BUILD, K_RANK_FINAL, K_LCP_FLAGS, K_CLUSTER,
    K_INVERT_COUNT, K_INVERT, K_SYNTH, K_FASTQ, K_BFS, K_CODEC, K_MISC, K_RESTORE, K_FQ_FORMAT, K_RO_KEYS, K_RO_GATHER,
    K_FQ_FORMAT_ORD, K_PERM_PACK, K_PERM_INVERT, K_POSBIN_L1, K_POSBIN_L2, K_POSBIN_APPLY,
    K_CMP_CHECK, K_CMP_COMPARE, K_CMP_EMIT, K_BGZF, K_DEFLATE, K_NUM
};
extern const char *const BFQ_KERNEL_NAMES[K_NUM];

struct ProfRec { int id; hipEvent_t a, b; double bytes; };

#define BFQ_IO_MAX_WORKERS 16
#define BFQ_IO_STAGE_BYTES (16u << 20)

struct DevCounters {
    u64 stats[8];
    u64 bigCount;
    u64 errSymbol;
    u64 errInvert;
    u64 errFreq3;
    u64 errTooLong;
    u64 tot[6];
    u64 mismatch;
    u64 nSegs;
    u64 errFastq;
    u64 hugeCount;
    u64 hugeRows;
    u64 bigClusters;
    u64 bigTotal;
    u64 pad[5];
};

struct RankIndex {
    u64 *lfq;
    u64 n;
};

struct CallState {
    bool piles = false;
    bool capped = false;
    u64 cappedPileRows = 0;
    bool keepRecs = false;
    const u64 *d_w12 = nullptr, *d_text3 = nullptr;
    size_t keepMark = 0;
    size_t writeHint = 0;
    bool arenaHeld = false;
    u8 *extBwt = nullptr, *extQual = nullptr;
    bool lcpScratch = false;
    std::function<void(u64, u64)> onRows;
};

struct bfq_ctx {
    int device = 0;
    hipStream_t stream = nullptr;
    hipStream_t copyStream = nullptr;
    hipStream_t copy() { if (!copyStream) HIP_CHECK(hipStreamCreateWithFlags(&copyStream, hipStreamNonBlocking)); return copyStream; }
    bfq_params P;
    BfqEnv env;
    std::string err;

    Arena ws;
    void reserve(size_t bytes);
    void wsFree();
    void adoptWorkspace(char *p, size_t bytes);
    void quiesce() { (void)hipStreamSynchronize(stream); }
    void reserveBegin(size_t bytes);
    void reserveJoin(bool adopt, size_t need);
    std::thread *wsThread = nullptr;
    char *wsPend = nullptr;
    size_t wsPendBytes = 0;
    double wsPendSecs = 0;
    void dropWorkspace();
    void *allocBytes(size_t bytes) { return ws.alloc(bytes); }
    template <class T> T *alloc(size_t count) { return (T *)allocBytes(count * sizeof(T)); }
    size_t mark() const { return ws.mark(); }
    void release(size_t m) { ws.release(m); }

    DevCounters *d_cnt = nullptr;
    DevCounters h_cnt;
    double *d_powtab = nullptr;
    double *d_qthr = nullptr;
    int qthrLo = 0, qthrN = 0;

    u8 *d_bwt = nullptr; u8 *d_qual = nullptr; u16 *d_lcp = nullptr;
    u32 *d_gcnt = nullptr;
    int gcntTerm = -1;
    u64 n = 0, N = 0;
    CallState call;
    size_t wsLimit() const { return env.wsCap ? (size_t)env.wsCap : (size_t)(P.ws_cap_mib > 0 ? P.ws_cap_mib : 0) << 20; }

    bool profOn = true;
    std::vector<hipEvent_t> evPool;
    size_t evUsed = 0;
    std::vector<ProfRec> recs;
    double profMs[K_NUM];
    u64 profLaunches[K_NUM];
    double profBytes[K_NUM];
    int profTraceId = -1;
    std::vector<float> profTrace;
    void profBegin(int id, double bytes);
    void profEnd();
    void profCollect();

    void sync();
    void fetchCounters();
    void zeroCounters();

    struct IoWorker { hipStream_t stream = nullptr; char *stage[2] = {nullptr, nullptr}; hipEvent_t done[2] = {nullptr, nullptr}; };
    IoWorker io[BFQ_IO_MAX_WORKERS];
    int ioWorkers = 0;
    void ioInit(int want);
    void ioFree();
    struct BfqWriter *writer = nullptr;

    u8 *d_text = nullptr;
    size_t textCap = 0;
    u8 *textBuf(size_t bytes);
    u64 residentLen = 0;
    bool residentValid = false;
    int residentParts = 0;
    u64 residentPstart[BFQ_MAX_PARTS + 1] = {0, 0, 0, 0, 0};
    u64 globN = 0;
    u64 globCounts[36] = {0};
};
using ScopedArena = ScopedArenaT<bfq_ctx>;

struct DevBuf {
    char *p = nullptr;
    DevBuf() = default;
    DevBuf(const DevBuf &) = delete; DevBuf &operator=(const DevBuf &) = delete;
    ~DevBuf() { free(); }
    bool tryAlloc(size_t bytes)
    {
        free();
        if (hipMalloc((void **)&p, bytes) == hipSuccess) return true;
        (void)hipGetLastError();
        p = nullptr;
        return false;
    }
    void alloc(size_t bytes, const char *what) { if (!tryAlloc(bytes)) throw BfqError{BFQ_E_NOMEM, std::string("device buffer for ") + what}; }
    void free() { if (p) (void)hipFree(p); p = nullptr; }
    char *release() { char *q = p; p = nullptr; return q; }
};
struct ScopedEvent {
    hipEvent_t e = nullptr;
    ScopedEvent() { HIP_CHECK(hipEventCreateWithFlags(&e, hipEventDisableTiming)); }
    ScopedEvent(const ScopedEvent &) = delete; ScopedEvent &operator=(const ScopedEvent &) = delete;
    ~ScopedEvent() { (void)hipEventDestroy(e); }
    operator hipEvent_t() const { return e; }
};

struct HostRef {
    void *ptr = nullptr; int fd = -1; u64 off = 0;
    bfq_outmap *om = nullptr;
    static HostRef mem(const void *p) { HostRef h; h.ptr = const_cast<void *>(p); return h; }
    static HostRef file(int fd, u64 off = 0) { HostRef h; h.fd = fd; h.off = off; return h; }
    bool null() const { return !ptr && fd < 0; }
};
void bfq_upload(bfq_ctx *c, void *d_dst, HostRef src, size_t len);
void bfq_download(bfq_ctx *c, HostRef dst, const void *d_src, size_t len);
struct TextSrc { HostRef ref; u64 len; };
struct TextMeasure {
    struct Part { bool bgzf = false; u64 raw = 0; u8 addNl = 0; std::vector<bfq_bgzf_member> dir; };
    Part part[BFQ_MAX_PARTS];
    int nparts = 0;
    u64 bound = 0, stage = 0;
    bool anyBgzf() const { return stage != 0; }
};
void bfq_text_measure(const TextSrc *parts, int nparts, TextMeasure *M);
void bfq_text_put(bfq_ctx *c, const TextSrc *parts, TextMeasure *M, u8 *d_dst, u8 *d_stage, u64 *pstart);
bool bfq_text_is_gzip(const TextSrc &t);
void bfq_upload(bfq_ctx *c, void *d_dst, const void *h_src, size_t len);
void bfq_download(bfq_ctx *c, void *h_dst, const void *d_src, size_t len);
void bfq_write_async(bfq_ctx *c, HostRef dst, const void *d_src, size_t len);
void bfq_write_wait(bfq_ctx *c);
struct BfqAsyncUpload;
BfqAsyncUpload *bfq_upload_begin(bfq_ctx *c, void *d_dst, HostRef src, size_t len);
void bfq_upload_join(BfqAsyncUpload *u);

struct OutFile {
    int fd = -1;
    bfq_outmap *m = nullptr;
    HostRef at(u64 off) const
    {
        if (!m) return HostRef::file(fd, off);
        HostRef h = HostRef::mem(bfq_outmap_ptr(m) + off);
        h.om = m; h.off = off;
        return h;
    }
    void open(int f, u64 mapLen, u64 prefault)
    {
        fd = f;
        if (f < 0) return;
        m = bfq_outmap_take(f, mapLen);
        if (m) bfq_outmap_extend(m, prefault);
        else m = bfq_outmap_open(f, mapLen, prefault);
    }
    bool close(u64 finalLen)
    {
        bool ok = true;
        if (m) ok = bfq_outmap_close(m, finalLen);
        else if (fd >= 0) ok = ftruncate(fd, (off_t)finalLen) == 0 || errno == EINVAL;
        m = nullptr;
        return ok;
    }
};

#define KLAUNCH(ctx, kid, bytes, kernel, grid, block, ...)                                     \
    do {                                                                                       \
        (ctx)->profBegin((kid), (double)(bytes));                                              \
        hipLaunchKernelGGL(kernel, dim3(grid), dim3(block), 0, (ctx)->stream, __VA_ARGS__);    \
        (ctx)->profEnd();                                                                      \
        HIP_CHECK(hipGetLastError());                                                          \
    } while (0)

template <class F> static int guarded(bfq_ctx *c, F body)
{
    if (!c) return BFQ_E_ARG;
    try {
        HIP_CHECK(hipSetDevice(c->device));
        c->err.clear();
        c->call = CallState{};
        body();
        return BFQ_OK;
    } catch (const BfqError &e) {
        c->err = e.msg;
        c->call = CallState{};
        (void)hipStreamSynchronize(c->stream);
        if (c->copyStream) (void)hipStreamSynchronize(c->copyStream);
        (void)hipGetLastError();
        c->recs.clear(); c->evUsed = 0;
        return e.code;
    } catch (const std::bad_alloc &) {
        c->err = "host out of memory";
        c->call = CallState{};
        return BFQ_E_NOMEM;
    }
}

static inline u64 ceil_div(u64 a, u64 b) { return (a + b - 1) / b; }
#define BFQ_MAX_GRID (1u << 19)
static inline unsigned bfq_grid(u64 items, u64 perBlock)
{
    u64 b = ceil_div(items, perBlock);
    return (unsigned)(b < 1 ? 1 : (b > BFQ_MAX_GRID ? BFQ_MAX_GRID : b));
}

struct SortRec { u32 *w0; u64 *w12; };

void bfq_exscan_u8(bfq_ctx *c, const u8 *in, u64 *out, u64 n, u64 *d_total);
void bfq_exscan_u32(bfq_ctx *c, const u32 *in, u64 *out, u64 n, u64 *d_total);
void bfq_exscan_u64(bfq_ctx *c, const u64 *in, u64 *out, u64 n, u64 *d_total);

u64 *bfq_line_index(bfq_ctx *c, const u8 *d_buf, u64 len, u64 *nlines);
u64 bfq_fastq_count_lines(bfq_ctx *c, const u8 *d_buf, u64 len);
u64 bfq_codec_bound(u64 n);
u64 bfq_codec_workspace(u64 n);
u64 bfq_codec_raw_len(const u8 *h_in, u64 len, u64 *nameWs = nullptr);
u64 bfq_codec_member_len(const u8 *h_in, u64 len);
u64 bfq_codec_compress_device(bfq_ctx *c, const u8 *d_in, u64 n, u8 *d_out, u64 cap);
u64 bfq_codec_decompress_device(bfq_ctx *c, const u8 *h_in, const u8 *d_in, u64 len, u8 *d_out, u64 cap);
u64 bfq_codec_checksum_device(bfq_ctx *c, const u8 *d_in, u64 n, u64 *d_tmp);
u64 bfq_rans_compress_device(bfq_ctx *c, const u8 *d_in, u64 n, u8 *d_out, u64 cap, bool dry);
u64 bfq_rans_decompress_device(bfq_ctx *c, const u8 *h_in, const u8 *d_in, u64 len, u8 *d_out, u64 cap);
u64 bfq_dnac_workspace(u64 n);
u64 bfq_dnac_compress_device(bfq_ctx *c, const u8 *d_in, u64 n, u8 *d_out, u64 cap, u64 *nbases);
u64 bfq_dnac_decompress_device(bfq_ctx *c, const u8 *h_in, const u8 *d_in, u64 len, u8 *d_out, u64 cap);
u64 bfq_dnac_member_len(const u8 *h_in, u64 len);
struct NamesSized { bool eligible = false; u64 nl = 0; const u64 *lineEnd = nullptr; u64 *offO = nullptr, *offN = nullptr, *offT = nullptr; u64 total[3] = {0, 0, 0}; };
bool bfq_names_size(bfq_ctx *c, const u8 *d_in, u64 n, NamesSized *S);
u64 bfq_names_sized_bytes(u64 n, u64 nl);
u64 bfq_names_rest_bytes(u64 n, const NamesSized &S);
u64 bfq_names_finish(bfq_ctx *c, const u8 *d_in, u64 n, const NamesSized &S, u32 flags, u8 *d_out, u64 cap);
u64 bfq_names_member_len(const u8 *h_in, u64 len);
u64 bfq_names_decode_extra(const u8 *h_in, u64 len, u64 *maxInner);
u64 bfq_names_decompress_device(bfq_ctx *c, const u8 *h_in, const u8 *d_in, u64 len, u8 *d_out, u64 cap);
u64 bfq_quals_workspace(u64 n, u64 nl);
u64 bfq_quals_finish(bfq_ctx *c, const u8 *d_in, u64 n, u32 flags, u8 *d_out, u64 cap);
u64 bfq_quals_member_len(const u8 *h_in, u64 len);
u64 bfq_quals_decompress_device(bfq_ctx *c, const u8 *h_in, const u8 *d_in, u64 len, u8 *d_out, u64 cap);
void bfq_codec_normalise(const u32 *cnt, u32 A, u16 *f);
u32 bfq_codec_bit_cost(u32 f);

void bfq_build_text(bfq_ctx *c, const u8 *d_bases, const u8 *d_quals, const u64 *d_roff, u64 N, u64 n,
                    u8 *T8, u8 *Q8, u64 *text3, u64 nwords);
#define BFQ_RS_BLOCK_ELEMS 98304
#define BFQ_RS_TILE 3072
static inline u64 bfq_radix_block_elems(u64 n)
{
    u64 tpb = BFQ_RS_BLOCK_ELEMS / BFQ_RS_TILE;
    while (tpb > 1 && n / (BFQ_RS_TILE * tpb) < 4096) tpb >>= 1;
    return BFQ_RS_TILE * tpb;
}
void bfq_build_keys(bfq_ctx *c, const u8 *T8, const u8 *Q8, const u64 *text3, u64 n, SortRec out, u32 *hist0);
SortRec bfq_radix_sort(bfq_ctx *c, SortRec in, SortRec tmp, u64 n, int passes = BFQ_KEY_PASSES, const u32 *hist0 = nullptr);
void bfq_refine(bfq_ctx *c, SortRec rec, const u64 *text3, u64 n, u16 *lcp, bfq_stats *st);
#define BFQ_HUGE_SEG 2048
void bfq_refine_huge(bfq_ctx *c, SortRec rec, const u64 *text3, u64 n, u16 *lcp, const u64 *hugeStart, const u64 *hugeLen);
void bfq_refine_bitonic(bfq_ctx *c, SortRec rec, const u64 *text3, u64 n, u16 *lcp, const u64 *d_start, const u64 *d_len, u64 count);
void bfq_emit_bwt(bfq_ctx *c, SortRec rec, u64 n, int termOut, u8 *bwt, u8 *qs, u32 *gcnt);
void bfq_step1_device(bfq_ctx *c, const u8 *d_bases, const u8 *d_quals, const u64 *d_roff, u64 N, u64 total,
                      int termOut, bfq_stats *st);
struct PileText { u8 *T8, *Q8; u64 *text3; };
void bfq_step1_piles(bfq_ctx *c, const u8 *d_bases, const u8 *d_quals, const u64 *d_roff, u64 N, u64 total, int termOut, bfq_stats *st,
                     const PileText *pre = nullptr, u64 capTarget = 0);
size_t bfq_ws_need_piles(u64 n, u64 N, u64 cap, u64 extra, bool lean = false);
struct PileRows { u64 m; u8 *bwt, *qs; u16 *lcp; const u64 *w12; };
u64 bfq_run_one_pile(bfq_ctx *c, const u8 *T8, const u8 *Q8, const u64 *text3, u64 n, u32 s, u32 s2, int termOut, PileRows *out);
void bfq_pile_pair_counts(bfq_ctx *c, const u8 *T8, u64 n, u64 *counts36);
void bfq_pack_text(bfq_ctx *c, const u8 *T8, u64 n, u64 *text3, u64 nwords);

RankIndex bfq_rank_build(bfq_ctx *c, const u8 *bwt, const u8 *qs, u64 n, int term, const u32 *gcnt = nullptr);
u64 *bfq_symbol_scans(bfq_ctx *c, const u8 *bwt, u64 n, int term, const u32 *gcntIn, u32 *gcntOut);
void bfq_rank_blocks(bfq_ctx *c, const u8 *bwt, u64 n, int term, const u64 *scanned, u64 *rank);
void bfq_lcp_flags(bfq_ctx *c, const u16 *lcp, u64 n, int K, u8 *in);
void bfq_lcp_from_bwt(bfq_ctx *c, const u8 *bwt, u64 n, u64 N, int term, u16 *lcp, u32 *gcntOut = nullptr,
                      const u64 *rankGiven = nullptr, u64 ringEntries = 0);
struct ClusterPos { const u64 *w12; const u64 *text3; u8 *outSym, *outQual; int B; u8 *editQual = nullptr, *repl = nullptr; };
struct ClusterRank { const u64 *rankBlk; u64 F[6]; u8 *qual, *repl; };
void bfq_clusters(bfq_ctx *c, const RankIndex &R, const u8 *bwt, const u8 *qual, const u8 *in, u64 n, const ClusterPos *pm = nullptr,
                  const ClusterRank *rm = nullptr);
#define BFQ_COMPACT_LCP_WIN (256ull << 20)
size_t bfq_ws_need_compact(bfq_ctx *c, u64 n, u64 N, u64 extra, bool haveLcp, size_t resident);
void bfq_steps234_compact(bfq_ctx *c, const u8 *bwt, u8 *qual, HostRef lcp, int lcp_bytes, u64 n, u64 N, u64 *d_roff, u32 *lens,
                          u8 **ob, u8 **oq, u64 extra, size_t resident);
void bfq_invert_count(bfq_ctx *c, const RankIndex &R, u64 N, u32 *lens);
void bfq_fixed_offsets(bfq_ctx *c, u64 N, u64 L, u64 *d_roff);
void bfq_invert(bfq_ctx *c, const RankIndex &R, u64 N, const u64 *d_roff, int B, u8 *out_bases, u8 *out_quals, u64 first = 0,
                u64 count = ~0ull, bool lines = false);
bool bfq_is_pinned(const void *p);
size_t bfq_posbins_need(u64 n);
void bfq_posbins(bfq_ctx *c, u64 *w12, const u8 *repl, const u8 *editQual, u64 n, const u64 *d_roff, u64 N, int B, u8 *outSym, u8 *outQual);

void bfq_synth_launch(bfq_ctx *c, const bfq_synth *s, u8 *d_bases, u8 *d_quals, u64 *d_roff);
u8 *bfq_synth_headers(bfq_ctx *c, const bfq_synth *s, u64 *len);

struct FqRec { u64 hdrStart, seqStart, qualStart; u32 hdrLen, len; };
struct DevFastq { u64 N, total; void *rec; u64 *roff; u8 *bases, *quals; u64 *lineEnd; };
void bfq_fastq_index(bfq_ctx *c, const u8 *d_fastq, u64 len, DevFastq *fq);
void bfq_fastq_parse(bfq_ctx *c, const u8 *d_fastq, u64 len, DevFastq *fq);
u64 bfq_fastq_format(bfq_ctx *c, const u8 *d_bases, const u8 *d_quals, const u64 *d_roff, u64 N, int mode, const u8 *d_hdr,
                     u64 hdrLen, const DevFastq *fq, u8 **d_out, u64 **recOffOut = nullptr, bool lines = false);
void bfq_fastq_hdr_stream(bfq_ctx *c, u64 N, const u8 *d_fastq, const DevFastq *fq, u8 **d_hdr, u64 *hdrLen, u64 **hOffOut = nullptr);
void bfq_fastq_format_lines(bfq_ctx *c, const u8 *d_dna, const u8 *d_qs, const u64 *d_roff, const u8 *d_hdr, const u64 *hStart,
                            const u32 *hLen, const u64 *recOff, u64 N, u64 outLen, u8 *d_out);
void bfq_fastq_format_ordered(bfq_ctx *c, const u8 *d_dna, const u8 *d_qs, const u64 *d_roff, const u8 *d_hdr, const u64 *hStart,
                              const u32 *hLen, const u64 *recOff, const u64 *inv, u64 N, u64 outLen, u8 *d_out);
void bfq_restore_sizes_ordered(bfq_ctx *c, const u32 *sizes, const u64 *inv, u64 N, u32 *sizesOut);
void bfq_fastq_part_index(bfq_ctx *c, const DevFastq *fq, const u64 *h_pstart, int nparts, u64 *d_idx);
void bfq_pick_u64(bfq_ctx *c, const u64 *d_src, const u64 *d_idx, int count, u64 addIdx, u64 *d_out);

struct EbwtLines { u8 *dna = nullptr, *qs = nullptr; u64 n = 0, N = 0; };
size_t bfq_ebwt_decode_need(const u8 *h_bwtz, u64 len_b, u64 len_q, size_t extraWs, bool keepLines);
void bfq_ebwt_decode_lines(bfq_ctx *c, const u8 *h_bwtz, u64 len_b, const u8 *h_qsz, u64 len_q, u8 *h_dna, u8 *h_qs, u64 cap,
                           uint64_t *stream_len, uint64_t *n_reads, size_t extraWs, EbwtLines *res);

struct RoText { const u8 *buf; const FqRec *rec; u64 len; };
void bfq_reorder_keys(bfq_ctx *c, const RoText *mates, int nmates, u64 N, int mode, int k, u64 seed, SortRec out);
void bfq_reorder_perm(bfq_ctx *c, SortRec sorted, const RoText *mates, int nmates, u64 N, u64 *perm, u64 *const *sizes);
void bfq_reorder_gather(bfq_ctx *c, const RoText &t, const u64 *perm, const u64 *newOff, u64 N, u8 *d_out);
void bfq_perm_pack(bfq_ctx *c, const u64 *perm, u64 N, u64 *d_words);
u64 bfq_perm_unpack_invert(bfq_ctx *c, const u64 *d_words, u64 N, u64 *perm, u64 *inv);
void bfq_reorder_sizes(bfq_ctx *c, const u64 *order, const RoText *mates, int nmates, u64 N, u64 *const *sizes);

struct CmpText { const u8 *buf; const FqRec *rec; };
void bfq_compare_check(bfq_ctx *c, CmpText A, CmpText B, const u64 *inv, u64 N, bfq_compare_report *d_rep, u64 *d_badRead);
void bfq_compare_pass(bfq_ctx *c, CmpText A, CmpText B, const u64 *inv, u64 N, u64 total, bfq_compare_report *d_rep, u32 *readDiffs);
void bfq_compare_emit(bfq_ctx *c, CmpText A, CmpText B, const u64 *inv, u64 N, u64 total, const u32 *readDiffs, const u64 *diffOff, u64 cap,
                      bfq_compare_diff *d_out);
```

bfqzip_amd/csrc/bfq_internal_host.h:

```cpp
#pragma once
#include <stdint.h>
#include <atomic>
#include <string>
#include "../../include/bfqzip_hip.h"

struct BfqError {
    int code;
    std::string msg;
};

struct BfqEnv {
    bool trace = false;
    int piles = 0;
    bool pilesSplit = false;
    bool noOverlap = false;
    bool noLengthGuess = false;
    bool posMode = false;
    bool posBins = true;
    int ioThreads = 0;
    int prefaultThreads = -1;
    unsigned long long hugeCap = 0;
    unsigned long long wsCap = 0;
    int device = -1;
    int fakeDevices = 0;
    bool lease = true;
    std::string leaseDir;
    bool compact = false;
    int dnaStatic = 0;
    int dnacK = 0, dnacH = 0, dnacW = 0, dnacSkip = -1;
    unsigned long long compactRing = 0;
    unsigned long long compactWin = 0;
    bool prefaultPause = false;
    unsigned long long bgzfBatch = 0;
    bool noOutmap = false;
};
BfqEnv bfq_env_read();
const BfqEnv &bfq_env();
int bfq_cpu_budget();
extern std::atomic<bool> g_bfqHipStarted;
extern std::atomic<int> g_bfqUploadsRunning;

struct bfq_outmap;
bfq_outmap *bfq_outmap_open(int fd, uint64_t map_len, uint64_t prefault_len);
bfq_outmap *bfq_outmap_take(int fd, uint64_t min_len);
char *bfq_outmap_ptr(bfq_outmap *m);
uint64_t bfq_outmap_len(bfq_outmap *m);
void bfq_outmap_extend(bfq_outmap *m, uint64_t prefault_len);
bool bfq_outmap_close(bfq_outmap *m, uint64_t final_len);
bool bfq_outmap_ensure(bfq_outmap *m, uint64_t off, uint64_t len);
int bfq_outmap_fd(bfq_outmap *m);
```

bfqzip_amd/csrc/k_radix.hip:

```cpp
#include "bfq_internal.h"
#include "bfq_device.h"

#ifndef RS_THREADS
#define RS_THREADS 256
#endif
#define RS_WAVES (RS_THREADS / 64)
#define RS_OCC (1024 / RS_THREADS)
#define RS_ROUNDS 12
#define RS_TILE (RS_THREADS * RS_ROUNDS)
static_assert(RS_TILE == BFQ_RS_TILE, "bfq_radix_block_elems() counts in scatter tiles");

template <class T>
__global__ __launch_bounds__(RS_THREADS) void k_radix_hist(const T *__restrict__ dw, u64 n, int shift,
                                                           u32 *__restrict__ hist, u64 nblocks, u64 blockElems)
{
    __shared__ u32 wh[RS_WAVES][256];
    u32 w = threadIdx.x >> 6;
    for (int i = threadIdx.x; i < RS_WAVES * 256; i += RS_THREADS) (&wh[0][0])[i] = 0;
    __syncthreads();
    u64 base = (u64)blockIdx.x * blockElems;
    u64 end = base + blockElems;
    if (end > n) end = n;
    constexpr int V = 16 / sizeof(T);
    u64 i = base + (u64)threadIdx.x * V;
    for (; i + V <= end; i += (u64)RS_THREADS * V) {
        uint4 x = *(const uint4 *)(dw + i);
        if (sizeof(T) == 4) {
            atomicAdd(&wh[w][(x.x >> shift) & 255u], 1u); atomicAdd(&wh[w][(x.y >> shift) & 255u], 1u);
            atomicAdd(&wh[w][(x.z >> shift) & 255u], 1u); atomicAdd(&wh[w][(x.w >> shift) & 255u], 1u);
        } else {
            atomicAdd(&wh[w][(x.x >> shift) & 255u], 1u); atomicAdd(&wh[w][(x.z >> shift) & 255u], 1u);
        }
    }
    for (; i < end; i++) {
        u32 d = (u32)(dw[i] >> shift) & 255u;
        atomicAdd(&wh[w][d], 1u);
    }
    __syncthreads();
    u32 d = threadIdx.x;
    if (d < 256) {
        u32 t = 0;
#pragma unroll
        for (int k = 0; k < RS_WAVES; k++) t += wh[k][d];
        hist[(u64)d * nblocks + blockIdx.x] = t;
    }
}

template <int DW>
__global__ __launch_bounds__(RS_THREADS, RS_OCC) void k_radix_scatter(SortRec in, SortRec out, u64 n, int shift,
                                                              const u64 *__restrict__ blockOff, u64 nblocks, u32 tilesPerBlock)
{
    __shared__ u64 stage[RS_TILE];
    __shared__ u8 dig[RS_TILE];
    __shared__ u32 wcnt[RS_WAVES][256];
    __shared__ u32 lstart[256];
    __shared__ u64 gbase[256];
    __shared__ u32 shscan[RS_WAVES];

    const u32 tid = threadIdx.x, lane = bfq_lane(), w = tid >> 6;
    const u64 ltmask = bfq_lanemask_lt();
    const u64 blk = blockIdx.x;
    if (tid < 256) gbase[tid] = blockOff[(u64)tid * nblocks + blk];

    for (u32 t = 0; t < tilesPerBlock; t++) {
        u64 tbase = (blk * tilesPerBlock + t) * RS_TILE;
        if (tbase >= n) break;
        u32 cnt = (n - tbase < (u64)RS_TILE) ? (u32)(n - tbase) : (u32)RS_TILE;

        for (int i = tid; i < RS_WAVES * 256; i += RS_THREADS) (&wcnt[0][0])[i] = 0;
        __syncthreads();

        u32 a0[RS_ROUNDS], a1[RS_ROUNDS], a2[RS_ROUNDS];
        u32 pk[RS_ROUNDS];
        const u32 lastSlot = cnt - 1;
#pragma unroll
        for (int r = 0; r < RS_ROUNDS; r++) {
            const u32 slot = w * (RS_ROUNDS * 64) + r * 64 + lane;
            const u64 src = tbase + (slot < lastSlot ? slot : lastSlot);
            a0[r] = in.w0[src];
            const u64 x12 = in.w12[src];
            a1[r] = (u32)x12;
            a2[r] = (u32)(x12 >> 32);
        }
#pragma unroll
        for (int r = 0; r < RS_ROUNDS; r++) {
            const u32 slot = w * (RS_ROUNDS * 64) + r * 64 + lane;
            if (slot >= cnt) { a0[r] = 0xFFFFFFFFu; a1[r] = 0xFFFFFFFFu; a2[r] = 0u; }
        }
#pragma unroll
        for (int r = 0; r < RS_ROUNDS; r++) {
            u32 d = ((DW ? a1[r] : a0[r]) >> shift) & 255u;
            u64 peers = ~0ull;
#pragma unroll
            for (int b = 0; b < 8; b++) {
                bool bit = (d >> b) & 1u;
                u64 bal = __ballot(bit);
                peers &= bit ? bal : ~bal;
            }
            u32 before = (u32)__popcll(peers & ltmask);
            u32 c0 = wcnt[w][d];
            pk[r] = (d << 16) | (c0 + before);
            bfq_wave_sync();
            if (before == 0) wcnt[w][d] = c0 + (u32)__popcll(peers);
            bfq_wave_sync();
        }
        __syncthreads();

        u32 tot = 0;
        if (tid < 256) {
#pragma unroll
            for (int k = 0; k < RS_WAVES; k++) { u32 ck = wcnt[k][tid]; wcnt[k][tid] = tot; tot += ck; }
        }
        {
            u32 inc = bfq_wave_incscan32_bp(tot);
            if (lane == 63) shscan[w] = inc;
            __syncthreads();
            u32 base = 0;
#pragma unroll
            for (int k = 0; k < RS_WAVES; k++) base += (k < (int)w) ? shscan[k] : 0u;
            if (tid < 256) lstart[tid] = base + inc - tot;
        }
        __syncthreads();

#pragma unroll
        for (int r = 0; r < RS_ROUNDS; r++) {
            u32 d = pk[r] >> 16;
            u32 p = lstart[d] + wcnt[w][d] + (pk[r] & 0xFFFFu);
            pk[r] = p;
            stage[p] = (u64)a0[r];
            dig[p] = (u8)d;
        }
        __syncthreads();
        u64 dst[RS_ROUNDS];
#pragma unroll
        for (int q = 0; q < RS_ROUNDS; q++) {
            u32 j = q * RS_THREADS + tid;
            u32 d = dig[j];
            dst[q] = gbase[d] + (u64)(j - lstart[d]);
            if (j < cnt) out.w0[dst[q]] = (u32)stage[j];
        }
        __syncthreads();
#pragma unroll
        for (int r = 0; r < RS_ROUNDS; r++) stage[pk[r]] = ((u64)a2[r] << 32) | a1[r];
        __syncthreads();
#pragma unroll
        for (int q = 0; q < RS_ROUNDS; q++) {
            u32 j = q * RS_THREADS + tid;
            if (j < cnt) out.w12[dst[q]] = stage[j];
        }
        __syncthreads();
        if (tid < 256) gbase[tid] += tot;
    }
}

SortRec bfq_radix_sort(bfq_ctx *c, SortRec in, SortRec tmp, u64 n, int passes, const u32 *hist0)
{
    if (n < 2) {
        if (n == 1 && (passes & 1)) {
            HIP_CHECK(hipMemcpyAsync(tmp.w0, in.w0, 4, hipMemcpyDeviceToDevice, c->stream));
            HIP_CHECK(hipMemcpyAsync(tmp.w12, in.w12, 8, hipMemcpyDeviceToDevice, c->stream));
        }
        return (passes & 1) ? tmp : in;
    }
    const u64 be = bfq_radix_block_elems(n);
    const u32 tpb = (u32)(be / RS_TILE);
    u64 nb = ceil_div(n, be);
    size_t m = c->mark();
    u32 *hist = c->alloc<u32>(256 * nb);
    u64 *off = c->alloc<u64>(256 * nb);
    SortRec out = tmp;
    for (int pass = 0; pass < passes; pass++) {
        const int dw = pass == 0 ? 1 : 0;
        const int shift = pass == 0 ? 24 : 8 * (pass - 1);
        const bool have = (pass == 0 && hist0);
        if (!have && dw)
            KLAUNCH(c, K_RADIX_HIST, 8.0 * (double)n, k_radix_hist<u64>, nb, RS_THREADS, (const u64 *)in.w12, n, shift, hist, nb, be);
        else if (!have)
            KLAUNCH(c, K_RADIX_HIST, 4.0 * (double)n, k_radix_hist<u32>, nb, RS_THREADS, (const u32 *)in.w0, n, shift, hist, nb, be);
        bfq_exscan_u32(c, have ? hist0 : hist, off, 256 * nb, nullptr);
        if (dw)
            KLAUNCH(c, K_RADIX_SCATTER, 24.0 * (double)n, k_radix_scatter<1>, nb, RS_THREADS, in, out, n, shift, (const u64 *)off, nb, tpb);
        else
            KLAUNCH(c, K_RADIX_SCATTER, 24.0 * (double)n, k_radix_scatter<0>, nb, RS_THREADS, in, out, n, shift, (const u64 *)off, nb, tpb);
        SortRec t = in; in = out; out = t;
    }
    c->release(m);
    return in;
}
```

bfqzip_amd/csrc/k_text.hip:

```cpp
#include "bfq_internal.h"
#include "bfq_device.h"

__device__ __forceinline__ u64 codes8(u64 x, bool *bad)
{
    u64 out = 0;
#pragma unroll
    for (int k = 0; k < 8; k++) {
        u32 c = (u32)(x >> (8 * k)) & 0xFFu;
        u32 h = (c >> 1) & 7u;
        u32 code = (0x40003521u >> (4 * h)) & 0xFu;
        u32 want = (u32)((0x4E00000047544341ull >> (8 * h)) & 0xFFu);
        if (c != want || code == 0) { *bad = true; code = 4; }
        out |= (u64)code << (8 * k);
    }
    return out;
}

__global__ __launch_bounds__(256) void k_text_from_reads(const u8 *__restrict__ bases, const u8 *__restrict__ quals,
                                                         const u64 *__restrict__ roff, u64 N, u8 *__restrict__ T8,
                                                         u8 *__restrict__ Q8, DevCounters *cnt)
{
    const u32 sub = threadIdx.x & 15u;
    u64 grp = ((u64)blockIdx.x * blockDim.x + threadIdx.x) >> 4;
    const u64 ngrp = ((u64)gridDim.x * blockDim.x) >> 4;
    bool bad = false, tooLong = false;
    for (u64 i = grp; i < N; i += ngrp) {
        u64 b = roff[i], e = roff[i + 1];
        u64 t0 = b + i, len = e - b;
        if (len > BFQ_MAX_READ_LEN) tooLong = true;
        if (len >= 8) {
            const u64 nw = (len + 7) >> 3;
            for (u64 j = sub; j < nw; j += 16) {
                const u64 k = (8 * j + 8 <= len) ? 8 * j : len - 8;
                u64 xb = *(const u64 *)(bases + b + k);
                u64 xq = *(const u64 *)(quals + b + k);
                *(u64 *)(T8 + t0 + k) = codes8(xb, &bad);
                *(u64 *)(Q8 + t0 + k) = xq;
            }
        } else if (sub == 0) {
            for (u64 j = 0; j < len; j++) {
                u32 code = bfq_base_code(bases[b + j]);
                if (code == BFQ_CODE_INVALID) { bad = true; code = 4; }
                T8[t0 + j] = (u8)code;
                Q8[t0 + j] = quals[b + j];
            }
        }
        if (sub == 0) { T8[t0 + len] = 0; Q8[t0 + len] = (u8)'#'; }
    }
    if (bad) atomicAdd(&cnt->errSymbol, 1ull);
    if (tooLong) atomicAdd(&cnt->errTooLong, 1ull);
}

__global__ __launch_bounds__(256) void k_pack3(const u8 *__restrict__ T8, u64 n, u64 *__restrict__ text3, u64 nwords)
{
    for (u64 w = (u64)blockIdx.x * blockDim.x + threadIdx.x; w < nwords; w += (u64)gridDim.x * blockDim.x) {
        u64 p0 = w * BFQ_SYMS_PER_WORD;
        u64 v = 0;
        if (p0 + 24 <= n) {
            u64 x[3] = {*(const u64 *)(T8 + p0), *(const u64 *)(T8 + p0 + 8), *(const u64 *)(T8 + p0 + 16)};
#pragma unroll
            for (int j = 0; j < BFQ_SYMS_PER_WORD; j++) v = (v << 3) | ((x[j >> 3] >> (8 * (j & 7))) & 7ull);
        } else {
#pragma unroll 1
            for (int j = 0; j < BFQ_SYMS_PER_WORD; j++) {
                u64 p = p0 + j;
                u64 c = (p < n) ? (u64)T8[p] : 0ull;
                v = (v << 3) | c;
            }
        }
        text3[bfq_t3_at(w)] = v;
        const u64 j = w / BFQ_T3_PER_SEC, r = w - j * BFQ_T3_PER_SEC;
        if (r < 2 && j) text3[(j - 1) * 8 + 6 + r] = v;
    }
}

__global__ __launch_bounds__(256) void k_build_keys(const u8 *__restrict__ T8, const u8 *__restrict__ Q8,
                                                    const u64 *__restrict__ text3, u64 n, SortRec out, u32 *__restrict__ hist0,
                                                    u64 nblocks, u64 blockElems)
{
    __shared__ u32 wh[4][256];
    const u32 w = threadIdx.x >> 6;
    const u32 sw = 1024 / BFQ_SYMS_PER_WORD, so = 1024 - sw * BFQ_SYMS_PER_WORD;
    for (u64 hb = blockIdx.x; hb < nblocks; hb += gridDim.x) {
        for (int i = threadIdx.x; i < 4 * 256; i += 256) (&wh[0][0])[i] = 0;
        __syncthreads();
        const u64 bbase = hb * blockElems;
        u64 bend = bbase + blockElems;
        if (bend > n) bend = n;
        u64 p0 = bbase + (u64)threadIdx.x * 4;
        u64 w0 = p0 / BFQ_SYMS_PER_WORD;
        u32 o0 = (u32)(p0 - w0 * BFQ_SYMS_PER_WORD);
        for (; p0 < bend; p0 += 1024) {
            u32 c4 = 0, q4 = 0;
            if (p0 >= 1 && p0 + 3 <= n) { c4 = *(const u32 *)(T8 + p0 - 1); q4 = *(const u32 *)(Q8 + p0 - 1); }
            else for (int k = 0; k < 4; k++) { u64 t = p0 + k; if (t >= 1 && t - 1 < n) { c4 |= (u32)T8[t - 1] << (8 * k); q4 |= (u32)Q8[t - 1] << (8 * k); } }
            const u64 *t3 = text3 + bfq_t3_at(w0);
            u64 t0 = t3[0], t1 = t3[1], t2 = t3[2];
            u32 rw0[4];
            u64 rw12[4];
            u64 wd = w0;
            u32 o = o0;
#pragma unroll
            for (int k = 0; k < 4; k++) {
                u64 a = (wd == w0) ? t0 : t1, bnext = (wd == w0) ? t1 : t2;
                u32 o3 = o * 3u;
                u64 hi = (a << o3) & BFQ_M63;
                u64 lo = o3 ? (bnext >> (63u - o3)) : 0ull;
                u64 sk = bfq_skey_of(bfq_mask_key(hi | lo));
                u32 pc = (c4 >> (8 * k)) & 0xFFu;
                u32 pq = pc ? (q4 >> (8 * k)) & 0xFFu : (u32)'#';
                u64 pay = bfq_pack_val(p0 + k, pc, pq);
                rw0[k] = bfq_rec_w0(sk);
                rw12[k] = ((u64)bfq_rec_w2(pay) << 32) | bfq_rec_w1(sk, pay);
                if (p0 + k < n) atomicAdd(&wh[w][(u32)sk & 255u], 1u);
                if (++o == BFQ_SYMS_PER_WORD) { o = 0; wd++; }
            }
            if (p0 + 4 <= n) {
                *(uint4 *)(out.w0 + p0) = make_uint4(rw0[0], rw0[1], rw0[2], rw0[3]);
                *(ulonglong2 *)(out.w12 + p0) = make_ulonglong2(rw12[0], rw12[1]);
                *(ulonglong2 *)(out.w12 + p0 + 2) = make_ulonglong2(rw12[2], rw12[3]);
            } else {
                for (int k = 0; p0 + k < n; k++) { out.w0[p0 + k] = rw0[k]; out.w12[p0 + k] = rw12[k]; }
            }
            w0 += sw; o0 += so;
            if (o0 >= BFQ_SYMS_PER_WORD) { o0 -= BFQ_SYMS_PER_WORD; w0++; }
        }
        __syncthreads();
        hist0[(u64)threadIdx.x * nblocks + hb] = wh[0][threadIdx.x] + wh[1][threadIdx.x] + wh[2][threadIdx.x] + wh[3][threadIdx.x];
        __syncthreads();
    }
}

void bfq_build_text(bfq_ctx *c, const u8 *d_bases, const u8 *d_quals, const u64 *d_roff, u64 N, u64 n, u8 *T8,
                    u8 *Q8, u64 *text3, u64 nwords)
{
    if (N) {
        u64 blocks = bfq_grid(N, 16);
        KLAUNCH(c, K_TEXT, 4.0 * (double)(n - N), k_text_from_reads, blocks, 256, d_bases, d_quals, d_roff, N, T8, Q8,
                c->d_cnt);
    }
    bfq_pack_text(c, T8, n, text3, nwords);
}


void bfq_pack_text(bfq_ctx *c, const u8 *T8, u64 n, u64 *text3, u64 nwords)
{
    const u64 nl = bfq_t3_logical(nwords);
    KLAUNCH(c, K_PACK, (double)n + 8.0 * (double)nwords, k_pack3, bfq_grid(nl, 256), 256, T8, n, text3, nl);
}

void bfq_build_keys(bfq_ctx *c, const u8 *T8, const u8 *Q8, const u64 *text3, u64 n, SortRec out, u32 *hist0)
{
    if (!n) return;
    const u64 be = bfq_radix_block_elems(n);
    const u64 nb = ceil_div(n, be);
    KLAUNCH(c, K_KEYS, 14.5 * (double)n, k_build_keys, bfq_grid(nb, 1), 256, T8, Q8, text3, n, out, hist0, nb, be);
}
```

include/bfqzip_hip.h:

```cpp
#ifndef BFQZIP_HIP_H
#define BFQZIP_HIP_H
#include <stdint.h>
#ifdef __cplusplus
extern "C" {
#endif

#define BFQ_OK              0
#define BFQ_E_ARG          -1
#define BFQ_E_HIP          -2
#define BFQ_E_SYMBOL       -3
#define BFQ_E_NOT_EBWT     -4
#define BFQ_E_TOO_LONG     -5
#define BFQ_E_FREQ3        -6
#define BFQ_E_NOMEM        -7
#define BFQ_E_IO           -8

#define BFQ_MAX_READ_LEN 65000

typedef struct bfq_params {
    int32_t K;
    int32_t m;
    int32_t v;
    int32_t f;
    int32_t t;
    int32_t term;
    int32_t M;
    int32_t B;
    int32_t ext;
    int32_t piles;
    int32_t ws_cap_mib;
    int32_t reserved[5];
} bfq_params;

typedef struct bfq_stats {
    uint64_t num_clust, num_clust_discarded, num_clust_amb_discarded, num_clust_mod,
             num_clust_alleq, bases_inside, qs_smoothed, modified;
    uint64_t n_rows, n_reads, n_segments, n_big_segments;
} bfq_stats;

typedef struct bfq_ctx bfq_ctx;

void     bfq_default_params(bfq_params *p);
bfq_ctx *bfq_create(int device, const bfq_params *p);
const char *bfq_create_error(void);
void     bfq_destroy(bfq_ctx *c);
int      bfq_set_params(bfq_ctx *c, const bfq_params *p);
const char *bfq_last_error(bfq_ctx *c);
void    *bfq_stream(bfq_ctx *c);
int      bfq_device_count(void);

int bfq_pick_device(char *info, int info_cap);
int bfq_device_lease(int n_slots, const char *const *slot_ids, int only_slot, char *path_out, int path_cap, double *waited_s);
int bfq_device_release(int slot);

void bfq_phase_enable(int on);
void bfq_phase(const char *name);
void bfq_phase_report(const char *tool);

int bfq_build_ebwt(bfq_ctx *c, const uint8_t *h_bases, const uint8_t *h_quals,
                   const uint64_t *h_read_off, uint64_t N, int term_out,
                   uint8_t *h_bwt, uint8_t *h_bwtqs, uint16_t *h_lcp16);

int bfq_count_reads(const uint8_t *h_bwt, uint64_t n, int term, uint64_t *N);
int bfq_smooth_invert(bfq_ctx *c, const uint8_t *h_bwt, const uint8_t *h_bwtqs,
                      const void *h_lcp, int lcp_bytes, uint64_t n,
                      uint8_t *h_out_bases, uint8_t *h_out_quals, uint64_t *h_out_read_off,
                      bfq_stats *st);

int bfq_run_reads(bfq_ctx *c, const uint8_t *h_bases, const uint8_t *h_quals,
                  const uint64_t *h_read_off, uint64_t N,
                  uint8_t *h_out_bases, uint8_t *h_out_quals, bfq_stats *st);

int bfq_run_reads_device(bfq_ctx *c, const uint8_t *d_bases, const uint8_t *d_quals,
                         const uint64_t *d_read_off, uint64_t N, uint64_t total,
                         uint8_t *d_out_bases, uint8_t *d_out_quals, bfq_stats *st);

uint64_t bfq_fastq_out_bound(uint64_t total_bases, uint64_t n_reads, uint64_t header_bytes);
int bfq_fastq_build_ebwt(bfq_ctx *c, const uint8_t *h_fastq, uint64_t len, int term_out,
                         uint8_t *h_bwt, uint8_t *h_bwtqs, uint16_t *h_lcp16, uint64_t cap_rows,
                         uint64_t *n_rows, uint64_t *n_reads);
int bfq_fastq_run(bfq_ctx *c, const uint8_t *h_fastq, uint64_t len, int keep_headers,
                  uint8_t *h_out, uint64_t cap, uint64_t *out_len, bfq_stats *st);
int bfq_fastq_run_streams(bfq_ctx *c, const uint8_t *h_fastq, uint64_t len,
                          uint8_t *h_dna, uint8_t *h_qs, uint64_t cap_stream, uint64_t *stream_len,
                          uint8_t *h_hdr, uint64_t cap_hdr, uint64_t *hdr_len, bfq_stats *st);
int bfq_smooth_invert_fastq(bfq_ctx *c, const uint8_t *h_bwt, const uint8_t *h_bwtqs,
                            const void *h_lcp, int lcp_bytes, uint64_t n,
                            const uint8_t *h_headers, uint64_t headers_len,
                            uint8_t *h_out, uint64_t cap, uint64_t *out_len, bfq_stats *st);

int bfq_fastq_build_ebwt_fd(bfq_ctx *c, int fastq_fd, uint64_t len, int term_out, int bwt_fd, int bwtqs_fd,
                            int lcp_fd, int lcp_bytes, uint64_t *n_rows, uint64_t *n_reads);
int bfq_smooth_invert_fastq_fd(bfq_ctx *c, int bwt_fd, int bwtqs_fd, int lcp_fd, int lcp_bytes, uint64_t n,
                               int headers_fd, uint64_t headers_len, int out_fd, uint64_t *out_len, bfq_stats *st);
int      bfq_output_prefault(int fd, uint64_t map_len, uint64_t prefault_len);
uint64_t bfq_fastq_rows_estimate(int fastq_fd, uint64_t len);

#define BFQ_MAX_PARTS 4
typedef struct bfq_text_part { const uint8_t *data; uint64_t len; } bfq_text_part;
typedef struct bfq_fastq_job {
    const bfq_text_part *parts; int32_t nparts;
    int32_t keep_headers;
    uint8_t *out_fastq; uint64_t cap_fastq;
    uint8_t *out_dna, *out_qs; uint64_t cap_stream;
    uint8_t *out_hdr; uint64_t cap_hdr;
    uint64_t fastq_len, stream_len, hdr_len, n_reads, total_bases;
    uint64_t part_reads[BFQ_MAX_PARTS + 1], part_fastq_off[BFQ_MAX_PARTS + 1],
             part_stream_off[BFQ_MAX_PARTS + 1], part_hdr_off[BFQ_MAX_PARTS + 1];
    int32_t  compress_streams;
    int32_t  name_codec;
    uint64_t dna_bytes, qs_bytes, hdr_bytes;
    int32_t  qual_codec;
    int32_t  reserved1;
} bfq_fastq_job;
int bfq_fastq_run_job(bfq_ctx *c, bfq_fastq_job *job, bfq_stats *st);

int bfq_glob_begin(bfq_ctx *c, const bfq_text_part *parts, int nparts, uint64_t *n_reads, uint64_t *total_bases);
int bfq_glob_local_text(bfq_ctx *c, uint8_t *d_T8, uint8_t *d_Q8);
int bfq_glob_pile_counts(bfq_ctx *c, const uint8_t *d_T8, uint64_t n, uint64_t *counts36);
int bfq_glob_init_out(bfq_ctx *c, const uint8_t *d_T8, const uint8_t *d_Q8, uint64_t n, uint8_t *d_sym, uint8_t *d_qual);
int bfq_glob_run_pile(bfq_ctx *c, const uint8_t *d_T8, const uint8_t *d_Q8, uint64_t n, int s, int s2,
                      uint8_t *d_sym, uint8_t *d_qual, bfq_stats *st);
int bfq_glob_finish(bfq_ctx *c, uint8_t *d_dna, uint8_t *d_qs, bfq_fastq_job *job);

void *bfq_host_alloc(uint64_t bytes);
void  bfq_host_free(void *p);

int     bfq_text_count_lines(const uint8_t *h_text, uint64_t len, uint64_t chunk, uint64_t *counts, int threads);
int     bfq_file_put(int fd, uint64_t offset, const void *src, uint64_t len, int threads);
void   *bfq_file_map(int fd, uint64_t offset, uint64_t len, int threads);
int     bfq_file_unmap(void *p, uint64_t offset, uint64_t len);
int64_t bfq_text_nth_newline(const uint8_t *h_text, uint64_t len, uint64_t k);

int bfq_fetch_ebwt(bfq_ctx *c, uint8_t *h_bwt, uint8_t *h_bwtqs, uint16_t *h_lcp16);

typedef struct bfq_synth {
    uint64_t seed;
    uint64_t N;
    uint32_t Lmin, Lmax;
    uint32_t coverage;
    uint32_t err_ppm;
    uint32_t n_ppm;
    uint32_t snp_every;
    uint32_t dsnp_every;
    uint32_t both_strands;
    uint64_t first;
    uint64_t collection;
    uint32_t reserved[2];
} bfq_synth;
void bfq_synth_default(bfq_synth *s, uint64_t N, uint32_t L);
uint64_t bfq_synth_total(const bfq_synth *s);
int bfq_synth_host(const bfq_synth *s, uint8_t *h_bases, uint8_t *h_quals, uint64_t *h_read_off);
int bfq_synth_device(bfq_ctx *c, const bfq_synth *s, uint8_t *d_bases, uint8_t *d_quals,
                     uint64_t *d_read_off);
int bfq_synth_fastq(bfq_ctx *c, const bfq_synth *s, uint8_t *h_out, uint64_t cap, uint64_t *out_len);

uint64_t bfq_stream_bound(uint64_t len);
int64_t  bfq_stream_raw_len(const uint8_t *h_in, uint64_t len);
int bfq_stream_compress(bfq_ctx *c, const uint8_t *h_in, uint64_t len, uint8_t *h_out, uint64_t cap, uint64_t *out_len);
int bfq_stream_decompress(bfq_ctx *c, const uint8_t *h_in, uint64_t len, uint8_t *h_out, uint64_t cap, uint64_t *out_len);
int bfq_names_compress(bfq_ctx *c, const uint8_t *h_in, uint64_t len, uint32_t flags, uint8_t *h_out, uint64_t cap, uint64_t *out_len);
int bfq_names_compress_device(bfq_ctx *c, const uint8_t *d_in, uint64_t len, uint32_t flags, uint8_t *d_out, uint64_t cap, uint64_t *out_len);
int bfq_quals_compress(bfq_ctx *c, const uint8_t *h_in, uint64_t len, uint32_t flags, uint8_t *h_out, uint64_t cap, uint64_t *out_len);
int bfq_quals_compress_device(bfq_ctx *c, const uint8_t *d_in, uint64_t len, uint32_t flags, uint8_t *d_out, uint64_t cap, uint64_t *out_len);
int bfq_stream_ebwt_decode(bfq_ctx *c, const uint8_t *h_bwtz, uint64_t len_b, const uint8_t *h_qsz, uint64_t len_q,
                           uint8_t *h_dna, uint8_t *h_qs, uint64_t cap, uint64_t *stream_len, uint64_t *n_reads);
int64_t bfq_fastq_restore_bound(const uint8_t *h_dna, uint64_t dna_len, const uint8_t *h_qs, uint64_t qs_len,
                                const uint8_t *h_hdr, uint64_t hdr_len);
int bfq_fastq_restore(bfq_ctx *c, const uint8_t *h_dna, uint64_t dna_len, const uint8_t *h_qs, uint64_t qs_len,
                      const uint8_t *h_hdr, uint64_t hdr_len, uint8_t *h_out, uint64_t cap, uint64_t *out_len, uint64_t *n_reads);
int bfq_fastq_restore_fd(bfq_ctx *c, int dna_fd, uint64_t dna_len, int qs_fd, uint64_t qs_len,
                         int hdr_fd, uint64_t hdr_len, int out_fd, uint64_t *out_len, uint64_t *n_reads);
typedef struct bfq_restore_group {
    uint64_t dna_off, dna_len;
    uint64_t qs_off,  qs_len;
    uint64_t hdr_off, hdr_len;
    uint64_t raw_stream;
    uint64_t raw_hdr;
    uint64_t reads;
    uint64_t text_bound;
} bfq_restore_group;
int64_t bfq_fastq_restore_groups(const uint8_t *h_dna, uint64_t dna_len, const uint8_t *h_qs, uint64_t qs_len,
                                 const uint8_t *h_hdr, uint64_t hdr_len,
                                 bfq_restore_group *groups, uint64_t cap, char *why, int why_cap);
int64_t bfq_stream_members(const uint8_t *h_in, uint64_t len);
int bfq_fastq_restore_grouped(bfq_ctx *c, const uint8_t *h_dna, uint64_t dna_len, const uint8_t *h_qs, uint64_t qs_len,
                              const uint8_t *h_hdr, uint64_t hdr_len, uint64_t first, uint64_t count,
                              uint8_t *h_out, uint64_t cap, uint64_t *out_len, uint64_t *n_reads);
int bfq_fastq_restore_grouped_fd(bfq_ctx *c, int dna_fd, uint64_t dna_len, int qs_fd, uint64_t qs_len, int hdr_fd, uint64_t hdr_len,
                                 uint64_t first, uint64_t count, int out_fd, uint64_t *out_len, uint64_t *n_reads);
typedef struct bfq_reorder_opts {
    int32_t  mode;
    int32_t  k;
    uint64_t seed;
    uint64_t reserved[2];
} bfq_reorder_opts;
uint64_t bfq_reorder_key(const uint8_t *seq, uint64_t len, int k);
int bfq_fastq_reorder(bfq_ctx *c, const bfq_text_part *parts, int nparts, const bfq_reorder_opts *opts, uint8_t *const *h_out,
                      const uint64_t *cap, uint64_t *out_len, uint64_t *h_perm, uint64_t *n_reads);
int bfq_fastq_reorder_fd(bfq_ctx *c, const int *in_fd, const uint64_t *in_len, int nparts, const bfq_reorder_opts *opts,
                         const int *out_fd, uint64_t *out_len, uint64_t *n_reads);
uint64_t bfq_perm_bound(uint64_t n_reads);
int64_t  bfq_perm_reads(const uint8_t *h_permz, uint64_t len);
int bfq_perm_encode(const uint64_t *h_perm, uint64_t N, const bfq_reorder_opts *opts, uint8_t *h_out, uint64_t cap, uint64_t *out_len);
int bfq_perm_decode(const uint8_t *h_permz, uint64_t len, uint64_t *h_perm, uint64_t cap_entries, uint64_t *N,
                    bfq_reorder_opts *opts_out, uint64_t *first_bad);
int bfq_fastq_reorder_keep(bfq_ctx *c, const bfq_text_part *parts, int nparts, const bfq_reorder_opts *opts, uint8_t *const *h_out,
                           const uint64_t *cap, uint64_t *out_len, uint8_t *h_permz, uint64_t cap_permz, uint64_t *permz_len,
                           uint64_t *n_reads);
int bfq_fastq_reorder_keep_fd(bfq_ctx *c, const int *in_fd, const uint64_t *in_len, int nparts, const bfq_reorder_opts *opts,
                              const int *out_fd, int perm_fd, uint64_t *out_len, uint64_t *permz_len, uint64_t *n_reads);
int bfq_fastq_unreorder(bfq_ctx *c, const bfq_text_part *parts, int nparts, const uint8_t *h_permz, uint64_t permz_len,
                        uint8_t *const *h_out, const uint64_t *cap, uint64_t *out_len, uint64_t *n_reads);
int bfq_fastq_unreorder_fd(bfq_ctx *c, const int *in_fd, const uint64_t *in_len, int nparts, int perm_fd, uint64_t permz_len,
                           const int *out_fd, uint64_t *out_len, uint64_t *n_reads);
int bfq_fastq_restore_ordered(bfq_ctx *c, const uint8_t *h_dna, uint64_t dna_len, const uint8_t *h_qs, uint64_t qs_len,
                              const uint8_t *h_hdr, uint64_t hdr_len, const uint8_t *h_permz, uint64_t permz_len,
                              uint8_t *h_out, uint64_t cap, uint64_t *out_len, uint64_t *n_reads);
int bfq_fastq_restore_ordered_fd(bfq_ctx *c, int dna_fd, uint64_t dna_len, int qs_fd, uint64_t qs_len, int hdr_fd, uint64_t hdr_len,
                                 int perm_fd, uint64_t permz_len, int out_fd, uint64_t *out_len, uint64_t *n_reads);
#define BFQ_CMP_SYMS 6
#define BFQ_CMP_POS  512
typedef struct bfq_compare_diff { uint64_t read; uint32_t pos; uint8_t base_a, base_b, qual_a, qual_b; } bfq_compare_diff;
typedef struct bfq_compare_report {
    uint64_t n_reads, total_bases;
    uint64_t n_diffs;
    uint64_t reads_changed, reads_bases_changed, reads_quals_changed;
    uint64_t bases_changed, quals_changed, quals_raised, quals_lowered;
    uint64_t qual_abs_sum, qual_sq_sum, qual_abs_max;
    uint64_t first_changed_read;
    uint64_t headers_same, headers_dropped, headers_changed;
    uint64_t subst[BFQ_CMP_SYMS * BFQ_CMP_SYMS];
    uint64_t qual_hist_a[256], qual_hist_b[256];
    uint64_t changed_base_qual_hist[256];
    uint64_t pos_len[BFQ_CMP_POS], pos_bases[BFQ_CMP_POS], pos_quals[BFQ_CMP_POS], pos_abs[BFQ_CMP_POS];
    uint64_t reserved[8];
} bfq_compare_report;
int bfq_fastq_compare   (bfq_ctx *c, const bfq_text_part *a, int na, const bfq_text_part *b, int nb,
                         const uint8_t *h_permz, uint64_t permz_len,
                         bfq_compare_report *rep, bfq_compare_diff *h_diffs, uint64_t cap_diffs);
int bfq_fastq_compare_fd(bfq_ctx *c, int a_fd, uint64_t a_len, int b_fd, uint64_t b_len, int perm_fd, uint64_t permz_len,
                         bfq_compare_report *rep, bfq_compare_diff *h_diffs, uint64_t cap_diffs);
typedef struct bfq_bgzf_member { uint64_t in_off, out_off; uint32_t in_len, out_len; } bfq_bgzf_member;
int bfq_bgzf_probe(const uint8_t *h, uint64_t len);
int bfq_bgzf_index(const uint8_t *h_in, uint64_t len, bfq_bgzf_member *m, uint64_t cap, uint64_t *n_members,
                   uint64_t *raw_len, uint64_t *bad_off);
int bfq_bgzf_inflate(bfq_ctx *c, const uint8_t *h_in, uint64_t len, uint8_t *h_out, uint64_t cap, uint64_t *out_len);
int bfq_bgzf_inflate_device(bfq_ctx *c, const uint8_t *h_in, uint64_t len, uint8_t *d_out, uint64_t cap, uint64_t *out_len);
int bfq_bgzf_inflate_fd(bfq_ctx *c, int in_fd, uint64_t len, int out_fd, uint64_t *out_len);
typedef struct bfq_gzip_stats { uint64_t members, pieces, decoders, chain, skipped, discarded; } bfq_gzip_stats;
int bfq_gzip_probe(const uint8_t *h, uint64_t len);
int bfq_gzip_measure(bfq_ctx *c, const uint8_t *h_in, uint64_t len, uint64_t chunk, uint64_t *raw_len, uint64_t *n_members, bfq_gzip_stats *stats);
int bfq_gzip_inflate(bfq_ctx *c, const uint8_t *h_in, uint64_t len, uint64_t chunk, uint8_t *h_out, uint64_t cap, uint64_t *out_len,
                     bfq_gzip_stats *stats);
int bfq_gzip_inflate_device(bfq_ctx *c, const uint8_t *h_in, uint64_t len, uint64_t chunk, uint8_t *d_out, uint64_t cap, uint64_t *out_len,
                            bfq_gzip_stats *stats);
int bfq_gzip_inflate_fd(bfq_ctx *c, int in_fd, uint64_t len, uint64_t chunk, int out_fd, uint64_t *out_len, bfq_gzip_stats *stats);
int bfq_gzip_inflate_host(const uint8_t *h_in, uint64_t len, uint64_t chunk, uint8_t *h_out, uint64_t cap, uint64_t *out_len,
                          bfq_gzip_stats *stats);
const char *bfq_gzip_host_error(void);
uint64_t bfq_bgzf_deflate_bound(uint64_t len);
int bfq_bgzf_deflate_host(const uint8_t *h_in, uint64_t len, int level, uint8_t *h_out, uint64_t cap, uint64_t *out_len);
int bfq_bgzf_deflate(bfq_ctx *c, const uint8_t *h_in, uint64_t len, int level, uint8_t *h_out, uint64_t cap, uint64_t *out_len);
int bfq_bgzf_deflate_device(bfq_ctx *c, const uint8_t *d_in, uint64_t len, int level, uint8_t *h_out, uint64_t cap, uint64_t *out_len);
int bfq_bgzf_deflate_fd(bfq_ctx *c, int in_fd, uint64_t len, int level, int out_fd, uint64_t *out_len);
int bfq_fastq_restore_bgzf_fd(bfq_ctx *c, int dna_fd, uint64_t dna_len, int qs_fd, uint64_t qs_len, int hdr_fd, uint64_t hdr_len,
                              int perm_fd, uint64_t permz_len, int level, int out_fd, uint64_t *out_len, uint64_t *raw_len,
                              uint64_t *n_reads);
int bfq_stream_reserve(bfq_ctx *c, uint64_t len);
int bfq_stream_compress_device(bfq_ctx *c, const uint8_t *d_in, uint64_t len, uint8_t *d_out, uint64_t cap, uint64_t *out_len);

int  bfq_prof_enable(bfq_ctx *c, int on);
void bfq_prof_reset(bfq_ctx *c);
int  bfq_prof_count(bfq_ctx *c);
int  bfq_posbin_geometry(uint64_t n_rows, uint64_t *window, int *bin_shift);
int  bfq_prof_get(bfq_ctx *c, int idx, char *name, int name_cap, double *total_ms,
                  uint64_t *launches, double *alg_bytes_total);
int     bfq_prof_trace_select(bfq_ctx *c, int idx);
int64_t bfq_prof_trace(bfq_ctx *c, float *ms, uint64_t cap);

uint64_t bfq_workspace_bytes(bfq_ctx *c);
const char *bfq_version(void);

#ifdef __cplusplus
}
#endif
#endif
```

Before: 11130.

## Fuse sort-key generation into the first radix scatter pass

Instead of materialising full key records and then sorting them, a count-only kernel builds the first-digit histogram from the packed text. The first scatter pass then regenerates each record on the fly from the tile's text, symbols and qualities, which it stages in LDS. This removes one full write and read of the record arrays (w0 plus w12 per suffix). The cost is extra arithmetic and LDS staging in the scatter kernel, and the text buffers are relocated. It is enabled by default and can be turned off with BFQ_FUSEKEYS.

```diff
diff --git a/bfqzip_amd/_lib.py b/bfqzip_amd/_lib.py
--- a/bfqzip_amd/_lib.py
+++ b/bfqzip_amd/_lib.py
@@ -16,7 +16,7 @@
     "bfq_text_count_lines", "bfq_text_nth_newline", "bfq_file_put", "bfq_file_map", "bfq_file_unmap", "bfq_fastq_build_ebwt_fd", "bfq_smooth_invert_fastq_fd",
     "bfq_glob_begin", "bfq_glob_local_text", "bfq_glob_pile_counts", "bfq_glob_init_out", "bfq_glob_run_pile", "bfq_glob_finish",
     "bfq_synth_default", "bfq_synth_total", "bfq_synth_host", "bfq_synth_device", "bfq_synth_fastq",
-    "bfq_posbin_geometry", "bfq_prof_enable", "bfq_prof_reset", "bfq_prof_count", "bfq_prof_get", "bfq_prof_trace_select", "bfq_prof_trace",
+    "bfq_posbin_geometry", "bfq_radix_geometry", "bfq_prof_enable", "bfq_prof_reset", "bfq_prof_count", "bfq_prof_get", "bfq_prof_trace_select", "bfq_prof_trace",
     "bfq_stream_bound", "bfq_stream_raw_len", "bfq_stream_compress", "bfq_stream_decompress",
     "bfq_stream_reserve", "bfq_stream_compress_device", "bfq_stream_ebwt_decode",
     "bfq_names_compress", "bfq_names_compress_device",
@@ -264,6 +264,7 @@
         L.bfq_gzip_host_error.argtypes = []
         L.bfq_fastq_restore_bgzf_fd.argtypes = [vp, C.c_int, u64, C.c_int, u64, C.c_int, u64, C.c_int, u64, C.c_int, C.c_int, pu64, pu64, pu64]
         L.bfq_posbin_geometry.argtypes = [u64, C.POINTER(u64), C.POINTER(C.c_int)]
+        L.bfq_radix_geometry.argtypes = [u64, C.POINTER(u64), C.POINTER(u64)]
         L.bfq_prof_enable.argtypes = [vp, C.c_int]
         L.bfq_prof_reset.argtypes = [vp]
         L.bfq_prof_count.argtypes = [vp]
diff --git a/bfqzip_amd/csrc/bfq_api.hip b/bfqzip_amd/csrc/bfq_api.hip
--- a/bfqzip_amd/csrc/bfq_api.hip
+++ b/bfqzip_amd/csrc/bfq_api.hip
@@ -279,6 +279,12 @@
     if (bin_shift) *bin_shift = s;
     return s >= 0 ? BFQ_OK : BFQ_E_ARG;
 }
+extern "C" int bfq_radix_geometry(uint64_t n_rows, uint64_t *tile_rows, uint64_t *block_rows)
+{
+    if (tile_rows) *tile_rows = BFQ_RS_TILE;
+    if (block_rows) *block_rows = bfq_radix_block_elems(n_rows);
+    return BFQ_OK;
+}
 extern "C" int bfq_prof_get(bfq_ctx *c, int idx, char *name, int cap, double *ms, uint64_t *launches, double *bytes)
 {
     if (!c || idx < 0 || idx >= K_NUM) return BFQ_E_ARG;
@@ -397,12 +403,19 @@
     B.w0 = c->alloc<u32>(n + 16);
     B.w12 = c->alloc<u64>(n + 16);
     if (bfq_env().trace) fprintf(stderr, "[bfq] sort buffers: A.w12 %p A.w0 %p B.w0 %p B.w12 %p (arena %p)\n", (void *)A.w12, (void *)A.w0, (void *)B.w0, (void *)B.w12, (void *)c->ws.base);
-    u8 *T8 = (u8 *)A.w0, *Q8 = (u8 *)A.w12;
+    const bool fuse = c->env.fuseKeys && n >= 2;
+    u8 *T8 = fuse ? (u8 *)B.w0 : (u8 *)A.w0, *Q8 = fuse ? (u8 *)B.w12 : (u8 *)A.w12;
     bfq_build_text(c, d_bases, d_quals, d_roff, N, n, T8, Q8, text3, nwords);
     u32 *hist0 = c->alloc<u32>(256 * ceil_div(n, bfq_radix_block_elems(n)));
     static_assert(BFQ_KEY_PASSES & 1, "an odd number of passes ends in the other buffer");
-    bfq_build_keys(c, T8, Q8, text3, n, B, hist0);
-    bfq_radix_sort(c, B, A, n, BFQ_KEY_PASSES, hist0);
+    if (fuse) {
+        const KeySrc gen{T8, Q8, text3};
+        bfq_count_keys(c, text3, n, hist0);
+        bfq_radix_sort(c, B, A, n, BFQ_KEY_PASSES, hist0, &gen);
+    } else {
+        bfq_build_keys(c, T8, Q8, text3, n, B, hist0);
+        bfq_radix_sort(c, B, A, n, BFQ_KEY_PASSES, hist0);
+    }
     c->release(mB);
     bfq_refine(c, A, text3, n, c->d_lcp, st);
     bfq_emit_bwt(c, A, n, termOut, c->d_bwt, c->d_qual, c->d_gcnt);
diff --git a/bfqzip_amd/csrc/bfq_device.h b/bfqzip_amd/csrc/bfq_device.h
--- a/bfqzip_amd/csrc/bfq_device.h
+++ b/bfqzip_amd/csrc/bfq_device.h
@@ -74,9 +74,8 @@
     return v + (row >= 1 ? t0 : 0ull) + (row >= 2 ? t1 : 0ull) + (row >= 3 ? t2 : 0ull);
 }
 
-__device__ __forceinline__ u32 bfq_wave_incscan32_bp(u32 v)
+__device__ __forceinline__ u32 bfq_wave_incscan32_bp(u32 v, u32 lane)
 {
-    u32 lane = bfq_lane();
 #pragma unroll
     for (int d = 1; d < 64; d <<= 1) {
         u32 t = (u32)__builtin_amdgcn_ds_bpermute(((int)lane - d) << 2, (int)v);
@@ -84,6 +83,8 @@
     }
     return v;
 }
+
+__device__ __forceinline__ u32 bfq_wave_incscan32_bp(u32 v) { return bfq_wave_incscan32_bp(v, bfq_lane()); }
 
 __device__ __forceinline__ u64 bfq_block_exscan64(u64 v, u64 *sh, u64 *total)
 {
diff --git a/bfqzip_amd/csrc/bfq_host.cpp b/bfqzip_amd/csrc/bfq_host.cpp
--- a/bfqzip_amd/csrc/bfq_host.cpp
+++ b/bfqzip_amd/csrc/bfq_host.cpp
@@ -50,6 +50,7 @@
         e.noLengthGuess = getenv("BFQ_NO_LENGTH_GUESS") != nullptr;
         e.posMode = geti("BFQ_POSMODE", 0) != 0;
         e.posBins = geti("BFQ_POSBINS", 1) != 0;
+        e.fuseKeys = geti("BFQ_FUSEKEYS", 1) != 0;
         e.ioThreads = geti("BFQ_IO_THREADS", 0);
         e.prefaultThreads = geti("BFQ_PREFAULT_THREADS", -1);
         e.hugeCap = getu("BFQ_HUGE_CAP", 0);
diff --git a/bfqzip_amd/csrc/bfq_internal.h b/bfqzip_amd/csrc/bfq_internal.h
--- a/bfqzip_amd/csrc/bfq_internal.h
+++ b/bfqzip_amd/csrc/bfq_internal.h
@@ -270,6 +270,7 @@
 }
 
 struct SortRec { u32 *w0; u64 *w12; };
+struct KeySrc { const u8 *T8, *Q8; const u64 *text3; };
 
 void bfq_exscan_u8(bfq_ctx *c, const u8 *in, u64 *out, u64 n, u64 *d_total);
 void bfq_exscan_u32(bfq_ctx *c, const u32 *in, u64 *out, u64 n, u64 *d_total);
@@ -316,7 +317,8 @@
     return BFQ_RS_TILE * tpb;
 }
 void bfq_build_keys(bfq_ctx *c, const u8 *T8, const u8 *Q8, const u64 *text3, u64 n, SortRec out, u32 *hist0);
-SortRec bfq_radix_sort(bfq_ctx *c, SortRec in, SortRec tmp, u64 n, int passes = BFQ_KEY_PASSES, const u32 *hist0 = nullptr);
+void bfq_count_keys(bfq_ctx *c, const u64 *text3, u64 n, u32 *hist0);
+SortRec bfq_radix_sort(bfq_ctx *c, SortRec in, SortRec tmp, u64 n, int passes = BFQ_KEY_PASSES, const u32 *hist0 = nullptr, const KeySrc *gen = nullptr);
 void bfq_refine(bfq_ctx *c, SortRec rec, const u64 *text3, u64 n, u16 *lcp, bfq_stats *st);
 #define BFQ_HUGE_SEG 2048
 void bfq_refine_huge(bfq_ctx *c, SortRec rec, const u64 *text3, u64 n, u16 *lcp, const u64 *hugeStart, const u64 *hugeLen);
diff --git a/bfqzip_amd/csrc/bfq_internal_host.h b/bfqzip_amd/csrc/bfq_internal_host.h
--- a/bfqzip_amd/csrc/bfq_internal_host.h
+++ b/bfqzip_amd/csrc/bfq_internal_host.h
@@ -17,6 +17,7 @@
     bool noLengthGuess = false;
     bool posMode = false;
     bool posBins = true;
+    bool fuseKeys = true;
     int ioThreads = 0;
     int prefaultThreads = -1;
     unsigned long long hugeCap = 0;
diff --git a/bfqzip_amd/csrc/bfq_keyrec.h b/bfqzip_amd/csrc/bfq_keyrec.h
--- /dev/null
+++ b/bfqzip_amd/csrc/bfq_keyrec.h
@@ -0,0 +1,83 @@
+#pragma once
+#include "bfq_common.h"
+
+BFQ_HD int bfq_clz32(u32 x)
+{
+#if defined(__HIP_DEVICE_COMPILE__)
+    return __clz((int)x);
+#else
+    return __builtin_clz(x);
+#endif
+}
+
+BFQ_HD void bfq_keyrec_halves(u64 a, u64 bnext, u32 o, u32 *hi, u32 *lo, u32 *len)
+{
+    const u32 o3 = o * 3u;
+    const u64 W = ((a << o3) & BFQ_M63) | (bnext >> (63u - o3));
+    u32 H = (u32)(W >> 39), L = (u32)(W >> 15) & 0xFFFFFFu;
+    const u32 F = 0x249249u;
+    const u32 zh = ~(H | (H >> 1) | (H >> 2)) & F, zl = ~(L | (L >> 1) | (L >> 2)) & F;
+    const u32 z = zh ? zh : zl;
+    u32 n = BFQ_KEY_SYMS;
+    if (z) {
+        const u32 b = 31u - (u32)bfq_clz32(z);
+        const u32 keep = 0u - (8u << b);
+        n = 7u - ((b * 11u) >> 5);
+        if (zh) { H &= keep; L = 0; }
+        else { L &= keep; n += 8u; }
+    }
+    *hi = H; *lo = L; *len = n;
+}
+
+BFQ_HD u32 bfq_keyrec_groups(u32 x)
+{
+    const u32 M7 = 0x1C71C7u;
+    const u32 A = (x >> 3) & M7, B = x & M7;
+    const u32 nz = (A | (A >> 1) | (A >> 2)) & 0x041041u;
+    const u32 S = A * 6u + B - nz * 5u;
+    const u32 v = (S & 0x03F03Fu) | ((S & 0xFC0FC0u) >> 1);
+    return (v & 0xFFFu) | ((v & 0xFFF000u) >> 2);
+}
+
+BFQ_HD u64 bfq_keyrec_skey(u64 a, u64 bnext, u32 o)
+{
+    u32 hi, lo, len;
+    bfq_keyrec_halves(a, bnext, o, &hi, &lo, &len);
+    return ((u64)bfq_keyrec_groups(hi) << 20) | (u64)bfq_keyrec_groups(lo) | ((u64)len << 40);
+}
+
+BFQ_HD u64 bfq_keyrec_pay(u64 pos, u32 prevCode, u32 prevQual)
+{
+    const u32 pc = pos ? (prevCode & 0xFFu) : 0u;
+    const u32 pq = pc ? (prevQual & 0xFFu) : (u32)'#';
+    return bfq_pack_val(pos, pc, pq);
+}
+
+BFQ_HD void bfq_keyrec(u64 a, u64 bnext, u32 o, u64 pos, u32 prevCode, u32 prevQual, u32 *w0, u64 *w12)
+{
+    u32 hi, lo, len;
+    bfq_keyrec_halves(a, bnext, o, &hi, &lo, &len);
+    const u32 kh = bfq_keyrec_groups(hi), kl = bfq_keyrec_groups(lo);
+    const u64 pay = bfq_keyrec_pay(pos, prevCode, prevQual);
+    *w0 = (kh << 12) | (kl >> 8);
+    const u32 w1 = (kl << 24) | (len << 16) | (u32)(pay >> 32);
+    *w12 = ((u64)bfq_rec_w2(pay) << 32) | w1;
+}
+
+BFQ_HD u32 bfq_keyrec_digit0(u64 a, u64 bnext, u32 o)
+{
+    u32 hi, lo, len;
+    bfq_keyrec_halves(a, bnext, o, &hi, &lo, &len);
+    return bfq_keyrec_groups(lo & 0xFFFu) & 255u;
+}
+
+BFQ_HD void bfq_keyrec_at(const u8 *T8, const u8 *Q8, const u64 *text3, u64 pos, u32 *w0, u64 *w12)
+{
+    const u64 w = pos / BFQ_SYMS_PER_WORD;
+    const u32 o = (u32)(pos - w * BFQ_SYMS_PER_WORD);
+    const u64 *t = text3 + bfq_t3_at(w);
+    bfq_keyrec(t[0], t[1], o, pos, pos ? T8[pos - 1] : 0u, pos ? Q8[pos - 1] : 0u, w0, w12);
+}
+
+BFQ_HD u32 bfq_div21_small(u32 q) { return (q * 3121u) >> 16; }
+BFQ_HD u32 bfq_div6_small(u32 e) { return (e * 171u) >> 10; }
diff --git a/bfqzip_amd/csrc/k_radix.hip b/bfqzip_amd/csrc/k_radix.hip
--- a/bfqzip_amd/csrc/k_radix.hip
+++ b/bfqzip_amd/csrc/k_radix.hip
@@ -1,5 +1,6 @@
 #include "bfq_internal.h"
 #include "bfq_device.h"
+#include "bfq_keyrec.h"
 
 #ifndef RS_THREADS
 #define RS_THREADS 256
@@ -8,6 +9,9 @@
 #define RS_OCC (1024 / RS_THREADS)
 #define RS_ROUNDS 12
 #define RS_TILE (RS_THREADS * RS_ROUNDS)
+#define GEN_PAD 16
+static_assert(RS_TILE / 16 <= RS_THREADS && (RS_TILE + 20) / BFQ_SYMS_PER_WORD + 2 <= RS_THREADS, "one text load per thread and array");
+static_assert(2 * (GEN_PAD + RS_TILE) + 8 * ((RS_TILE + 20) / BFQ_SYMS_PER_WORD + 2) <= 8 * RS_TILE && RS_TILE + 20 < 4096, "the tile's text fits the staging buffer");
 static_assert(RS_TILE == BFQ_RS_TILE, "bfq_radix_block_elems() counts in scatter tiles");
 
 template <class T>
@@ -46,11 +50,12 @@
     }
 }
 
-template <int DW>
+template <int DW, bool GEN>
 __global__ __launch_bounds__(RS_THREADS, RS_OCC) void k_radix_scatter(SortRec in, SortRec out, u64 n, int shift,
-                                                              const u64 *__restrict__ blockOff, u64 nblocks, u32 tilesPerBlock)
+                                                              const u64 *__restrict__ blockOff, u64 nblocks, u32 tilesPerBlock,
+                                                              KeySrc src)
 {
-    __shared__ u64 stage[RS_TILE];
+    __shared__ __attribute__((aligned(16))) u64 stage[RS_TILE];
     __shared__ u8 dig[RS_TILE];
     __shared__ u32 wcnt[RS_WAVES][256];
     __shared__ u32 lstart[256];
@@ -66,26 +71,63 @@
         u64 tbase = (blk * tilesPerBlock + t) * RS_TILE;
         if (tbase >= n) break;
         u32 cnt = (n - tbase < (u64)RS_TILE) ? (u32)(n - tbase) : (u32)RS_TILE;
-
-        for (int i = tid; i < RS_WAVES * 256; i += RS_THREADS) (&wcnt[0][0])[i] = 0;
-        __syncthreads();
-
-        u32 a0[RS_ROUNDS], a1[RS_ROUNDS], a2[RS_ROUNDS];
+        u32 tid0 = tid;
+        if (GEN) asm volatile("" : "+v"(tid0));
+        const u32 ln = GEN ? (tid0 & 63u) : lane, wv = GEN ? (tid0 >> 6) : w;
+        const u64 ltm = GEN ? ((1ull << ln) - 1ull) : ltmask;
+        const u32 slot0 = wv * (RS_ROUNDS * 64) + ln;
+
+        for (int i = tid0; i < RS_WAVES * 256; i += RS_THREADS) (&wcnt[0][0])[i] = 0;
+        u8 *const tL = (u8 *)stage, *const qL = tL + GEN_PAD + RS_TILE;
+        const u64 *const wL = (const u64 *)(qL + GEN_PAD + RS_TILE);
+        const u64 wb = tbase / BFQ_SYMS_PER_WORD;
+        const u32 ob = (u32)(tbase - wb * BFQ_SYMS_PER_WORD);
+        if (GEN) {
+            if (tid0 < RS_TILE / 16 && 16 * tid0 < cnt) {
+                *(uint4 *)(tL + GEN_PAD + 16 * tid0) = *(const uint4 *)(src.T8 + tbase + 16 * tid0);
+                *(uint4 *)(qL + GEN_PAD + 16 * tid0) = *(const uint4 *)(src.Q8 + tbase + 16 * tid0);
+            }
+            if (tid0 == RS_THREADS - 1 && tbase) { tL[GEN_PAD - 1] = src.T8[tbase - 1]; qL[GEN_PAD - 1] = src.Q8[tbase - 1]; }
+            const u64 sb = wb / BFQ_T3_PER_SEC;
+            const u32 rb = (u32)(wb - sb * BFQ_T3_PER_SEC);
+            const u32 nw = bfq_div21_small(ob + cnt - 1) + 2;
+            if (tid0 < nw) {
+                const u32 e = rb + tid0, es = bfq_div6_small(e);
+                ((u64 *)wL)[tid0] = src.text3[sb * 8 + es * 8 + (e - es * BFQ_T3_PER_SEC)];
+            }
+        }
+        __syncthreads();
+
+        u32 a0[RS_ROUNDS], a1[RS_ROUNDS], a2[GEN ? 1 : RS_ROUNDS];
         u32 pk[RS_ROUNDS];
         const u32 lastSlot = cnt - 1;
+        if (GEN) {
+#pragma unroll
+            for (int r = 0; r < RS_ROUNDS; r++) {
+                const u32 slot = slot0 + r * 64;
+                const u32 s = slot < lastSlot ? slot : lastSlot;
+                const u32 dq = bfq_div21_small(ob + s);
+                u64 x12;
+                bfq_keyrec(wL[dq], wL[dq + 1], ob + s - dq * BFQ_SYMS_PER_WORD, tbase + s, tL[GEN_PAD - 1 + s], qL[GEN_PAD - 1 + s], &a0[r], &x12);
+                a1[r] = (u32)x12;
+                if (slot >= cnt) { a0[r] = 0xFFFFFFFFu; a1[r] = 0xFFFFFFFFu; }
+                __builtin_amdgcn_sched_barrier(0);
+            }
+        } else {
+#pragma unroll
+            for (int r = 0; r < RS_ROUNDS; r++) {
+                const u32 slot = slot0 + r * 64;
+                const u64 row = tbase + (slot < lastSlot ? slot : lastSlot);
+                a0[r] = in.w0[row];
+                const u64 x12 = in.w12[row];
+                a1[r] = (u32)x12;
+                a2[r] = (u32)(x12 >> 32);
+            }
+        }
 #pragma unroll
         for (int r = 0; r < RS_ROUNDS; r++) {
-            const u32 slot = w * (RS_ROUNDS * 64) + r * 64 + lane;
-            const u64 src = tbase + (slot < lastSlot ? slot : lastSlot);
-            a0[r] = in.w0[src];
-            const u64 x12 = in.w12[src];
-            a1[r] = (u32)x12;
-            a2[r] = (u32)(x12 >> 32);
-        }
-#pragma unroll
-        for (int r = 0; r < RS_ROUNDS; r++) {
-            const u32 slot = w * (RS_ROUNDS * 64) + r * 64 + lane;
-            if (slot >= cnt) { a0[r] = 0xFFFFFFFFu; a1[r] = 0xFFFFFFFFu; a2[r] = 0u; }
+            const u32 slot = slot0 + r * 64;
+            if (!GEN && slot >= cnt) { a0[r] = 0xFFFFFFFFu; a1[r] = 0xFFFFFFFFu; a2[r] = 0u; }
         }
 #pragma unroll
         for (int r = 0; r < RS_ROUNDS; r++) {
@@ -97,35 +139,35 @@
                 u64 bal = __ballot(bit);
                 peers &= bit ? bal : ~bal;
             }
-            u32 before = (u32)__popcll(peers & ltmask);
-            u32 c0 = wcnt[w][d];
+            u32 before = (u32)__popcll(peers & ltm);
+            u32 c0 = wcnt[wv][d];
             pk[r] = (d << 16) | (c0 + before);
             bfq_wave_sync();
-            if (before == 0) wcnt[w][d] = c0 + (u32)__popcll(peers);
+            if (before == 0) wcnt[wv][d] = c0 + (u32)__popcll(peers);
             bfq_wave_sync();
         }
         __syncthreads();
 
         u32 tot = 0;
-        if (tid < 256) {
-#pragma unroll
-            for (int k = 0; k < RS_WAVES; k++) { u32 ck = wcnt[k][tid]; wcnt[k][tid] = tot; tot += ck; }
+        if (tid0 < 256) {
+#pragma unroll
+            for (int k = 0; k < RS_WAVES; k++) { u32 ck = wcnt[k][tid0]; wcnt[k][tid0] = tot; tot += ck; }
         }
         {
-            u32 inc = bfq_wave_incscan32_bp(tot);
-            if (lane == 63) shscan[w] = inc;
+            u32 inc = GEN ? bfq_wave_incscan32_bp(tot, ln) : bfq_wave_incscan32_bp(tot);
+            if (ln == 63) shscan[wv] = inc;
             __syncthreads();
             u32 base = 0;
 #pragma unroll
-            for (int k = 0; k < RS_WAVES; k++) base += (k < (int)w) ? shscan[k] : 0u;
-            if (tid < 256) lstart[tid] = base + inc - tot;
+            for (int k = 0; k < RS_WAVES; k++) base += (k < (int)wv) ? shscan[k] : 0u;
+            if (tid0 < 256) lstart[tid0] = base + inc - tot;
         }
         __syncthreads();
 
 #pragma unroll
         for (int r = 0; r < RS_ROUNDS; r++) {
             u32 d = pk[r] >> 16;
-            u32 p = lstart[d] + wcnt[w][d] + (pk[r] & 0xFFFFu);
+            u32 p = lstart[d] + wcnt[wv][d] + (pk[r] & 0xFFFFu);
             pk[r] = p;
             stage[p] = (u64)a0[r];
             dig[p] = (u8)d;
@@ -134,27 +176,28 @@
         u64 dst[RS_ROUNDS];
 #pragma unroll
         for (int q = 0; q < RS_ROUNDS; q++) {
-            u32 j = q * RS_THREADS + tid;
+            u32 j = q * RS_THREADS + tid0;
             u32 d = dig[j];
             dst[q] = gbase[d] + (u64)(j - lstart[d]);
             if (j < cnt) out.w0[dst[q]] = (u32)stage[j];
         }
         __syncthreads();
 #pragma unroll
-        for (int r = 0; r < RS_ROUNDS; r++) stage[pk[r]] = ((u64)a2[r] << 32) | a1[r];
+        for (int r = 0; r < RS_ROUNDS; r++) stage[pk[r]] = ((u64)(GEN ? (u32)tbase + slot0 + r * 64 : a2[r]) << 32) | a1[r];
         __syncthreads();
 #pragma unroll
         for (int q = 0; q < RS_ROUNDS; q++) {
-            u32 j = q * RS_THREADS + tid;
+            u32 j = q * RS_THREADS + tid0;
             if (j < cnt) out.w12[dst[q]] = stage[j];
         }
         __syncthreads();
-        if (tid < 256) gbase[tid] += tot;
+        if (tid0 < 256) gbase[tid0] += tot;
     }
 }
 
-SortRec bfq_radix_sort(bfq_ctx *c, SortRec in, SortRec tmp, u64 n, int passes, const u32 *hist0)
+SortRec bfq_radix_sort(bfq_ctx *c, SortRec in, SortRec tmp, u64 n, int passes, const u32 *hist0, const KeySrc *gen)
 {
+    if (gen && (!hist0 || n < 2 || passes < 1)) throw BfqError{BFQ_E_ARG, "bfq_radix_sort: a generating first pass needs its counts and two rows"};
     if (n < 2) {
         if (n == 1 && (passes & 1)) {
             HIP_CHECK(hipMemcpyAsync(tmp.w0, in.w0, 4, hipMemcpyDeviceToDevice, c->stream));
@@ -178,10 +221,12 @@
         else if (!have)
             KLAUNCH(c, K_RADIX_HIST, 4.0 * (double)n, k_radix_hist<u32>, nb, RS_THREADS, (const u32 *)in.w0, n, shift, hist, nb, be);
         bfq_exscan_u32(c, have ? hist0 : hist, off, 256 * nb, nullptr);
-        if (dw)
-            KLAUNCH(c, K_RADIX_SCATTER, 24.0 * (double)n, k_radix_scatter<1>, nb, RS_THREADS, in, out, n, shift, (const u64 *)off, nb, tpb);
+        if (pass == 0 && gen)
+            KLAUNCH(c, K_RADIX_SCATTER, 14.51 * (double)n, (k_radix_scatter<1, true>), nb, RS_THREADS, in, out, n, shift, (const u64 *)off, nb, tpb, *gen);
+        else if (dw)
+            KLAUNCH(c, K_RADIX_SCATTER, 24.0 * (double)n, (k_radix_scatter<1, false>), nb, RS_THREADS, in, out, n, shift, (const u64 *)off, nb, tpb, KeySrc{});
         else
-            KLAUNCH(c, K_RADIX_SCATTER, 24.0 * (double)n, k_radix_scatter<0>, nb, RS_THREADS, in, out, n, shift, (const u64 *)off, nb, tpb);
+            KLAUNCH(c, K_RADIX_SCATTER, 24.0 * (double)n, (k_radix_scatter<0, false>), nb, RS_THREADS, in, out, n, shift, (const u64 *)off, nb, tpb, KeySrc{});
         SortRec t = in; in = out; out = t;
     }
     c->release(m);
diff --git a/bfqzip_amd/csrc/k_text.hip b/bfqzip_amd/csrc/k_text.hip
--- a/bfqzip_amd/csrc/k_text.hip
+++ b/bfqzip_amd/csrc/k_text.hip
@@ -1,5 +1,6 @@
 #include "bfq_internal.h"
 #include "bfq_device.h"
+#include "bfq_keyrec.h"
 
 __device__ __forceinline__ u64 codes8(u64 x, bool *bad)
 {
@@ -74,6 +75,7 @@
     }
 }
 
+template <bool COUNT>
 __global__ __launch_bounds__(256) void k_build_keys(const u8 *__restrict__ T8, const u8 *__restrict__ Q8,
                                                     const u64 *__restrict__ text3, u64 n, SortRec out, u32 *__restrict__ hist0,
                                                     u64 nblocks, u64 blockElems)
@@ -92,8 +94,10 @@
         u32 o0 = (u32)(p0 - w0 * BFQ_SYMS_PER_WORD);
         for (; p0 < bend; p0 += 1024) {
             u32 c4 = 0, q4 = 0;
-            if (p0 >= 1 && p0 + 3 <= n) { c4 = *(const u32 *)(T8 + p0 - 1); q4 = *(const u32 *)(Q8 + p0 - 1); }
-            else for (int k = 0; k < 4; k++) { u64 t = p0 + k; if (t >= 1 && t - 1 < n) { c4 |= (u32)T8[t - 1] << (8 * k); q4 |= (u32)Q8[t - 1] << (8 * k); } }
+            if (!COUNT) {
+                if (p0 >= 1 && p0 + 3 <= n) { c4 = *(const u32 *)(T8 + p0 - 1); q4 = *(const u32 *)(Q8 + p0 - 1); }
+                else for (int k = 0; k < 4; k++) { u64 t = p0 + k; if (t >= 1 && t - 1 < n) { c4 |= (u32)T8[t - 1] << (8 * k); q4 |= (u32)Q8[t - 1] << (8 * k); } }
+            }
             const u64 *t3 = text3 + bfq_t3_at(w0);
             u64 t0 = t3[0], t1 = t3[1], t2 = t3[2];
             u32 rw0[4];
@@ -103,23 +107,20 @@
 #pragma unroll
             for (int k = 0; k < 4; k++) {
                 u64 a = (wd == w0) ? t0 : t1, bnext = (wd == w0) ? t1 : t2;
-                u32 o3 = o * 3u;
-                u64 hi = (a << o3) & BFQ_M63;
-                u64 lo = o3 ? (bnext >> (63u - o3)) : 0ull;
-                u64 sk = bfq_skey_of(bfq_mask_key(hi | lo));
-                u32 pc = (c4 >> (8 * k)) & 0xFFu;
-                u32 pq = pc ? (q4 >> (8 * k)) & 0xFFu : (u32)'#';
-                u64 pay = bfq_pack_val(p0 + k, pc, pq);
-                rw0[k] = bfq_rec_w0(sk);
-                rw12[k] = ((u64)bfq_rec_w2(pay) << 32) | bfq_rec_w1(sk, pay);
-                if (p0 + k < n) atomicAdd(&wh[w][(u32)sk & 255u], 1u);
+                u32 d0;
+                if (COUNT) d0 = bfq_keyrec_digit0(a, bnext, o);
+                else {
+                    bfq_keyrec(a, bnext, o, p0 + k, (c4 >> (8 * k)) & 0xFFu, (q4 >> (8 * k)) & 0xFFu, &rw0[k], &rw12[k]);
+                    d0 = (u32)rw12[k] >> 24;
+                }
+                if (p0 + k < n) atomicAdd(&wh[w][d0], 1u);
                 if (++o == BFQ_SYMS_PER_WORD) { o = 0; wd++; }
             }
-            if (p0 + 4 <= n) {
+            if (!COUNT && p0 + 4 <= n) {
                 *(uint4 *)(out.w0 + p0) = make_uint4(rw0[0], rw0[1], rw0[2], rw0[3]);
                 *(ulonglong2 *)(out.w12 + p0) = make_ulonglong2(rw12[0], rw12[1]);
                 *(ulonglong2 *)(out.w12 + p0 + 2) = make_ulonglong2(rw12[2], rw12[3]);
-            } else {
+            } else if (!COUNT) {
                 for (int k = 0; p0 + k < n; k++) { out.w0[p0 + k] = rw0[k]; out.w12[p0 + k] = rw12[k]; }
             }
             w0 += sw; o0 += so;
@@ -154,5 +155,14 @@
     if (!n) return;
     const u64 be = bfq_radix_block_elems(n);
     const u64 nb = ceil_div(n, be);
-    KLAUNCH(c, K_KEYS, 14.5 * (double)n, k_build_keys, bfq_grid(nb, 1), 256, T8, Q8, text3, n, out, hist0, nb, be);
+    KLAUNCH(c, K_KEYS, 14.5 * (double)n, k_build_keys<false>, bfq_grid(nb, 1), 256, T8, Q8, text3, n, out, hist0, nb, be);
 }
+
+void bfq_count_keys(bfq_ctx *c, const u64 *text3, u64 n, u32 *hist0)
+{
+    if (!n) return;
+    const u64 be = bfq_radix_block_elems(n);
+    const u64 nb = ceil_div(n, be);
+    KLAUNCH(c, K_KEYS, 0.51 * (double)n + 1024.0 * (double)nb, k_build_keys<true>, bfq_grid(nb, 1), 256, (const u8 *)nullptr, (const u8 *)nullptr, text3, n,
+            SortRec{}, hist0, nb, be);
+}
diff --git a/include/bfqzip_hip.h b/include/bfqzip_hip.h
--- a/include/bfqzip_hip.h
+++ b/include/bfqzip_hip.h
@@ -274,6 +274,7 @@
 void bfq_prof_reset(bfq_ctx *c);
 int  bfq_prof_count(bfq_ctx *c);
 int  bfq_posbin_geometry(uint64_t n_rows, uint64_t *window, int *bin_shift);
+int  bfq_radix_geometry(uint64_t n_rows, uint64_t *tile_rows, uint64_t *block_rows);
 int  bfq_prof_get(bfq_ctx *c, int idx, char *name, int name_cap, double *total_ms,
                   uint64_t *launches, double *alg_bytes_total);
 int     bfq_prof_trace_select(bfq_ctx *c, int idx);
```

After: 11610, median of 6. 4.2% higher.
